# datafusion-contrib/orc-rust

Measured on AMD Instinct MI355X. Metric: decoded GB/s + Mrows/s into Arrow, TPC-H lineitem stripe, higher is better.
Workload: dtype int64/i128/u8

## Files before the change

include/orcgpu.h:

```cpp
#ifndef ORCGPU_H
#define ORCGPU_H

#include <stddef.h>
#include <stdint.h>

#ifdef __cplusplus
extern "C" {
#endif

enum {
  ORCGPU_OK = 0,
  ORCGPU_IO_ERROR = 1,
  ORCGPU_OUT_OF_SPEC = 2,
  ORCGPU_VARINT_TOO_LARGE = 3,
  ORCGPU_DECODE_TIMESTAMP = 4,
  ORCGPU_OFFSET_OVERFLOW = 5,
  ORCGPU_MISMATCHED_SCHEMA = 6,
  ORCGPU_UNSUPPORTED = 7,
  ORCGPU_ARROW = 8,
  ORCGPU_BUILD_DECODER = 9,
  ORCGPU_UNEXPECTED = 10,
  ORCGPU_HIP_ERROR = 100,
  ORCGPU_INVALID_ARGUMENT = 101,
  ORCGPU_END_OF_FILE = 110
// ... 231 lines not shown
int orcgpu_reader_set_device_output(orcgpu_reader* r, int on);
int orcgpu_reader_next_batch_device(orcgpu_reader* r, struct ArrowDeviceArray* out_array, struct ArrowSchema* out_schema);
int orcgpu_reader_d2h_bytes(const orcgpu_reader* r, uint64_t* bytes);
uint64_t orcgpu_result_buffer_bytes(const orcgpu_result* r);
int orcgpu_reader_reads_ahead(orcgpu_reader* r);
int orcgpu_device_array_wait(const struct ArrowDeviceArray* array, void* hip_stream);
int orcgpu_device_array_dlpack(const struct ArrowDeviceArray* array, uint32_t column, int buffer, void** out_managed_tensor);
int orcgpu_unpack_bits(orcgpu_ctx* ctx, const void* d_bits, uint64_t n, uint8_t* d_bytes, void* hip_stream);

#define ORCGPU_ENC_ON_DEVICE 1u
int orcgpu_encode_rle2(orcgpu_ctx* ctx, const void* values, uint64_t n, int int_bytes, int is_signed, uint32_t flags, uint8_t* out, uint64_t out_cap,
                       uint64_t* out_len);
int orcgpu_encode_rle2_i64(orcgpu_ctx* ctx, const int64_t* values, uint64_t n, int is_signed, uint8_t* out, uint64_t out_cap, uint64_t* out_len);
int orcgpu_encode_byte_rle(orcgpu_ctx* ctx, const void* values, uint64_t n, uint32_t flags, uint8_t* out, uint64_t out_cap, uint64_t* out_len);
int orcgpu_encode_boolean(orcgpu_ctx* ctx, const void* bits, uint64_t n_bits, uint32_t flags, uint8_t* out, uint64_t out_cap, uint64_t* out_len);

typedef struct orcgpu_enc_column {
  int32_t arrow_type;
  uint32_t flags;
  uint64_t n_rows;
  const uint8_t* validity;
  const void* values;
  const void* offsets;
} orcgpu_enc_column;
typedef struct orcgpu_enc_stream {
  int32_t kind;
  uint32_t pad;
  const uint8_t* data;
  uint64_t len;
} orcgpu_enc_stream;
int orcgpu_encode_column(orcgpu_ctx* ctx, const orcgpu_enc_column* col, orcgpu_enc_stream streams[3], uint32_t* n_streams);
int orcgpu_encode_fetch(orcgpu_ctx* ctx, const orcgpu_enc_stream* stream, uint8_t* out);

typedef struct orcgpu_writer orcgpu_writer;
typedef struct orcgpu_writer_opts {
  uint32_t batch_size;
  uint32_t pad;
  uint64_t stripe_byte_size;
} orcgpu_writer_opts;
typedef struct orcgpu_writer_counts {
  uint64_t stripes, rows;
  uint64_t bytes;
  uint64_t round_trips;
  uint64_t stripe_round_trips;
  uint64_t nested_slices;
  uint64_t nested_gathers;
} orcgpu_writer_counts;
int orcgpu_writer_open_file(orcgpu_ctx* ctx, const char* path, const struct ArrowSchema* schema, const orcgpu_writer_opts* opts, orcgpu_writer** out);
int orcgpu_writer_open_bytes(orcgpu_ctx* ctx, const struct ArrowSchema* schema, const orcgpu_writer_opts* opts, orcgpu_writer** out);
int orcgpu_writer_write(orcgpu_writer* w, const struct ArrowSchema* schema, const struct ArrowArray* batch, uint32_t flags);
int orcgpu_writer_flush_stripe(orcgpu_writer* w);
int orcgpu_writer_close(orcgpu_writer* w);
int orcgpu_writer_take_bytes(orcgpu_writer* w, uint8_t* out, uint64_t cap, uint64_t* len);
int orcgpu_writer_stats(const orcgpu_writer* w, orcgpu_writer_counts* out);
uint64_t orcgpu_writer_stripe_rows(const orcgpu_writer* w, uint64_t stripe);
void orcgpu_writer_free(orcgpu_writer* w);

int orcgpu_writer_set_compression(orcgpu_writer* w, int kind, uint64_t block_size);
int orcgpu_compress_stream(orcgpu_ctx* ctx, int kind, uint64_t block_size, const void* in, uint64_t n, uint32_t flags, uint8_t* out, uint64_t out_cap,
                           uint64_t* out_len);

int orcgpu_writer_set_row_index(orcgpu_writer* w, uint64_t stride);

int orcgpu_writer_set_dictionary(orcgpu_writer* w, double key_size_threshold);
int orcgpu_writer_dictionary_counts(const orcgpu_writer* w, uint64_t* dictionary, uint64_t* direct);

int orcgpu_writer_set_bloom_filter(orcgpu_writer* w, const char* const* columns, uint32_t n_columns, double fpp);

int orcgpu_last_timing(const orcgpu_ctx* ctx, float* total_ms, float* expand_ms, uint32_t* expand_launches);
#define ORCGPU_N_PHASES 7
int orcgpu_last_phase_ms(const orcgpu_ctx* ctx, float* ms, uint32_t n);

typedef struct orcgpu_lane_stats {
  uint32_t lane, n_lanes;
  uint64_t stream_bytes, arrow_bytes;
  float start_ms, total_ms;
  float phase_ms[ORCGPU_N_PHASES];
  float seq_kernel_ms, exec_kernel_ms;
  float walk_short_kernel_ms, dict_emit_kernel_ms;
  float literals_kernel_ms;
} orcgpu_lane_stats;
int orcgpu_last_lane_stats(const orcgpu_ctx* ctx, uint32_t lane, orcgpu_lane_stats* out);

#ifdef __cplusplus
}
#endif
#endif
```

orc_rust_amd/capi.py:

```python
import ctypes as C
import os

import numpy as np

from . import build as _build

OK = 0
ERR_NAMES = {
    0: "Ok", 1: "IoError", 2: "OutOfSpec", 3: "VarintTooLarge", 4: "DecodeTimestamp", 5: "OffsetOverflow", 6: "MismatchedSchema",
    7: "UnsupportedTypeVariant", 8: "Arrow", 9: "BuildDecoder", 10: "Unexpected", 100: "HipError", 101: "InvalidArgument",
}
COMP = {"none": 0, "zlib": 1, "snappy": 2, "lzo": 3, "lz4": 4, "zstd": 5}
EXPORTS = [
    "orcgpu_open", "orcgpu_close", "orcgpu_last_error", "orcgpu_version", "orcgpu_abi_version", "orcgpu_stage_stripe", "orcgpu_staged_free",
    "orcgpu_staged_bytes", "orcgpu_decode_staged", "orcgpu_stripe_decode", "orcgpu_result_free", "orcgpu_result_status",
    "orcgpu_result_rows", "orcgpu_result_batches", "orcgpu_result_arrow_bytes", "orcgpu_result_batch_view",
    "orcgpu_result_copy_batch", "orcgpu_result_fetch", "orcgpu_result_fetch_async", "orcgpu_result_select", "orcgpu_selection_batches", "orcgpu_timezone_offsets", "orcgpu_result_export_batch", "orcgpu_last_timing", "orcgpu_last_phase_ms", "orcgpu_last_lane_stats", "orcgpu_encode_rle2_i64", "orcgpu_encode_rle2", "orcgpu_encode_byte_rle", "orcgpu_encode_boolean", "orcgpu_encode_column", "orcgpu_encode_fetch",
    "orcgpu_reader_open_file", "orcgpu_reader_open_bytes", "orcgpu_reader_close", "orcgpu_reader_set_batch_size",
    "orcgpu_reader_set_projection", "orcgpu_reader_set_projection_roots", "orcgpu_reader_set_schema", "orcgpu_reader_set_byte_range", "orcgpu_reader_set_shard", "orcgpu_shard_columns", "orcgpu_reader_column_weight", "orcgpu_reader_set_timestamp_precision", "orcgpu_reader_set_row_selection", "orcgpu_reader_set_prefetch",
    "orcgpu_reader_set_row_group_pruning", "orcgpu_reader_row_groups", "orcgpu_index_entry", "orcgpu_reader_set_predicate",
    "orcgpu_predicate_row_groups",
    "orcgpu_result_filter", "orcgpu_reader_set_row_filter", "orcgpu_reader_filter_rows",
    "orcgpu_reader_total_rows", "orcgpu_reader_stripe_count", "orcgpu_reader_column_count", "orcgpu_reader_column_name",
    "orcgpu_reader_next_batch",
    "orcgpu_result_export_batch_device", "orcgpu_reader_set_device_output", "orcgpu_reader_next_batch_device", "orcgpu_reader_d2h_bytes",
    "orcgpu_device_array_wait", "orcgpu_device_array_dlpack", "orcgpu_unpack_bits", "orcgpu_result_buffer_bytes", "orcgpu_reader_reads_ahead",
    "orcgpu_writer_open_file", "orcgpu_writer_open_bytes", "orcgpu_writer_write", "orcgpu_writer_flush_stripe", "orcgpu_writer_close",
    "orcgpu_writer_take_bytes", "orcgpu_writer_stats", "orcgpu_writer_stripe_rows", "orcgpu_writer_free",
    "orcgpu_writer_set_compression", "orcgpu_compress_stream", "orcgpu_writer_set_row_index",
    "orcgpu_writer_set_dictionary", "orcgpu_writer_dictionary_counts",
    "orcgpu_writer_set_bloom_filter",
]


class OrcGpuError(RuntimeError):
    def __init__(self, code, msg=""):
        super().__init__("%s (%d): %s" % (ERR_NAMES.get(code, "?"), code, msg))
        self.code = code


class StreamEntry(C.Structure):
    _fields_ = [("chunk_offset", C.c_uint64), ("skip_bytes", C.c_uint32), ("skip_values", C.c_uint32), ("skip_bits", C.c_uint32)]


class Stream(C.Structure):
    _fields_ = [("column_id", C.c_uint32), ("kind", C.c_int32), ("ptr", C.c_void_p), ("len", C.c_uint64),
                ("skip_bytes", C.c_uint32), ("skip_values", C.c_uint32), ("entries", C.c_void_p), ("n_entries", C.c_uint32), ("skip_bits", C.c_uint32)]


class Column(C.Structure):
    _fields_ = [("column_id", C.c_uint32), ("orc_type", C.c_int32), ("encoding", C.c_int32), ("dictionary_size", C.c_uint32),
                ("precision", C.c_uint32), ("scale", C.c_uint32), ("arrow_target", C.c_int32), ("arrow_precision", C.c_uint32),
                ("arrow_scale", C.c_uint32), ("parent", C.c_uint32)]


class StripeDesc(C.Structure):
    _fields_ = [("n_rows", C.c_uint64), ("compression", C.c_int32), ("block_size", C.c_uint64), ("ts_base_seconds", C.c_int64),
                ("batch_size", C.c_uint32), ("n_streams", C.c_uint32), ("streams", C.POINTER(Stream)), ("n_columns", C.c_uint32),
                ("columns", C.POINTER(Column)), ("writer_timezone", C.c_char_p)]


class LaneStats(C.Structure):
    _fields_ = [("lane", C.c_uint32), ("n_lanes", C.c_uint32), ("stream_bytes", C.c_uint64), ("arrow_bytes", C.c_uint64),
                ("start_ms", C.c_float), ("total_ms", C.c_float), ("phase_ms", C.c_float * 7), ("seq_kernel_ms", C.c_float),
                ("exec_kernel_ms", C.c_float), ("walk_short_kernel_ms", C.c_float), ("dict_emit_kernel_ms", C.c_float),
                ("literals_kernel_ms", C.c_float)]


class RowSelector(C.Structure):
    _fields_ = [("row_count", C.c_uint64), ("skip", C.c_int32)]


def selector_array(selectors):
    arr = (RowSelector * max(1, len(selectors)))()
    for i, (n, skip) in enumerate(selectors):
        arr[i].row_count = n
        arr[i].skip = 1 if skip else 0
    return arr


def selection_batches(selectors, stripe_rows, batch_size=8192):
    L = load()
    cap = len(selectors) + stripe_rows // max(1, batch_size) + 8
    starts, lens = (C.c_uint64 * cap)(), (C.c_uint32 * cap)()
    rest = (RowSelector * (len(selectors) + 2))()
    n_out, n_rest = C.c_uint32(), C.c_uint32()
    rc = L.orcgpu_selection_batches(selector_array(selectors), len(selectors), stripe_rows, batch_size, starts, lens, cap, C.byref(n_out), rest,
                                    len(selectors) + 2, C.byref(n_rest))
    assert rc == 0 and n_out.value <= cap
    return [(starts[i], lens[i]) for i in range(n_out.value)], [(rest[i].row_count, bool(rest[i].skip)) for i in range(n_rest.value)]


def timezone_offsets(name, instants):
    L = load()
    a = np.ascontiguousarray(instants, dtype=np.int64)
    out = np.zeros(len(a), dtype=np.int32)
    epoch = C.c_int64()
    rc = L.orcgpu_timezone_offsets(name.encode(), a.ctypes.data_as(C.c_void_p), len(a), out.ctypes.data_as(C.c_void_p), C.byref(epoch))
    if rc:
        raise OrcGpuError(rc, "time zone %r" % name)
# ... 19 lines not shown


ENC_ON_DEVICE = 1
ARROW = {"bool": 10, "int8": 11, "int16": 12, "int32": 13, "int64": 14, "float32": 15, "float64": 16, "utf8": 17, "binary": 18,
         "large_utf8": 25, "large_binary": 26}


class BatchView(C.Structure):
    _fields_ = [("length", C.c_uint64), ("null_count", C.c_uint64), ("validity", C.c_void_p), ("values", C.c_void_p),
                ("values_bytes", C.c_uint64), ("offsets", C.c_void_p)]


_lib = None
ABI_VERSION = 4


def lib_path():
    return _build.SO


def load():
    global _lib
    if _lib is not None:
        return _lib
    so = os.environ.get("ORCGPU_LIB") or _build.build()
    os.environ.setdefault("GPU_MAX_HW_QUEUES", "8")
    if "TZDIR" not in os.environ and not os.path.isdir("/usr/share/zoneinfo"):
        try:
            import tzdata
            os.environ["TZDIR"] = os.path.join(os.path.dirname(tzdata.__file__), "zoneinfo")
        except ImportError:
            pass
    L = C.CDLL(so)
    L.orcgpu_open.restype = C.c_void_p
    L.orcgpu_open.argtypes = [C.c_int, C.c_void_p]
    L.orcgpu_close.argtypes = [C.c_void_p]
    L.orcgpu_last_error.restype = C.c_char_p
    L.orcgpu_last_error.argtypes = [C.c_void_p]
    L.orcgpu_version.restype = C.c_char_p
    if L.orcgpu_abi_version() != ABI_VERSION:
        raise RuntimeError("liborcgpu.so speaks ABI %d, this binding %d (include/orcgpu.h: ORCGPU_ABI_VERSION)" % (L.orcgpu_abi_version(), ABI_VERSION))
    L.orcgpu_stage_stripe.argtypes = [C.c_void_p, C.POINTER(StripeDesc), C.POINTER(C.c_void_p)]
    L.orcgpu_staged_free.argtypes = [C.c_void_p]
    L.orcgpu_staged_bytes.restype = C.c_uint64
    L.orcgpu_staged_bytes.argtypes = [C.c_void_p]
    L.orcgpu_decode_staged.argtypes = [C.c_void_p, C.POINTER(C.c_void_p), C.c_uint32, C.POINTER(C.c_void_p)]
    L.orcgpu_stripe_decode.argtypes = [C.c_void_p, C.POINTER(StripeDesc), C.POINTER(C.c_void_p)]
    L.orcgpu_result_free.argtypes = [C.c_void_p]
    L.orcgpu_result_status.argtypes = [C.c_void_p, C.POINTER(C.c_uint32), C.POINTER(C.c_uint32)]
    L.orcgpu_result_rows.restype = C.c_uint64
    L.orcgpu_result_rows.argtypes = [C.c_void_p]
    L.orcgpu_result_batches.restype = C.c_uint32
    L.orcgpu_result_batches.argtypes = [C.c_void_p]
    L.orcgpu_result_arrow_bytes.restype = C.c_uint64
    L.orcgpu_result_arrow_bytes.argtypes = [C.c_void_p]
    L.orcgpu_result_batch_view.argtypes = [C.c_void_p, C.c_uint32, C.c_uint32, C.POINTER(BatchView)]
    L.orcgpu_result_copy_batch.argtypes = [C.c_void_p, C.c_void_p, C.c_uint32, C.c_uint32, C.c_void_p, C.c_void_p, C.c_void_p]
    L.orcgpu_result_fetch.argtypes = [C.c_void_p, C.c_void_p]
    L.orcgpu_result_fetch_async.argtypes = [C.c_void_p, C.c_void_p]
    L.orcgpu_reader_set_prefetch.argtypes = [C.c_void_p, C.c_uint32]
    L.orcgpu_reader_set_shard.argtypes = [C.c_void_p, C.c_uint32, C.c_uint32, C.c_int]
    L.orcgpu_shard_columns.argtypes = [C.POINTER(C.c_double), C.c_uint32, C.c_uint32, C.POINTER(C.c_uint32)]
    L.orcgpu_reader_column_weight.argtypes = [C.c_void_p, C.c_uint32]
    L.orcgpu_reader_column_weight.restype = C.c_double
    from .predicate import ColumnIndex, PredicateNode
    L.orcgpu_reader_set_predicate.argtypes = [C.c_void_p, C.POINTER(PredicateNode), C.c_uint32]
    L.orcgpu_predicate_row_groups.argtypes = [C.POINTER(PredicateNode), C.c_uint32, C.POINTER(ColumnIndex), C.c_uint32, C.c_uint64, C.c_uint64,
                                              C.c_void_p, C.POINTER(C.c_uint32)]
    L.orcgpu_result_filter.argtypes = [C.c_void_p, C.c_void_p, C.POINTER(PredicateNode), C.c_uint32, C.POINTER(C.c_char_p), C.c_uint32,
                                       C.POINTER(C.c_uint64)]
    L.orcgpu_reader_set_row_filter.argtypes = [C.c_void_p, C.POINTER(PredicateNode), C.c_uint32]
    L.orcgpu_reader_filter_rows.argtypes = [C.c_void_p, C.POINTER(C.c_uint64), C.POINTER(C.c_uint64)]
    L.orcgpu_reader_set_row_group_pruning.argtypes = [C.c_void_p, C.c_int]
    L.orcgpu_reader_row_groups.argtypes = [C.c_void_p, C.POINTER(C.c_uint64), C.POINTER(C.c_uint64)]
    L.orcgpu_index_entry.argtypes = [C.POINTER(Column), C.c_int, C.c_int, C.POINTER(C.c_uint64), C.c_uint32, C.c_int32, C.POINTER(StreamEntry)]
    L.orcgpu_result_select.argtypes = [C.c_void_p, C.c_void_p, C.POINTER(RowSelector), C.c_uint32]
    L.orcgpu_selection_batches.argtypes = [C.POINTER(RowSelector), C.c_uint32, C.c_uint64, C.c_uint32, C.POINTER(C.c_uint64), C.POINTER(C.c_uint32),
                                           C.c_uint32, C.POINTER(C.c_uint32), C.POINTER(RowSelector), C.c_uint32, C.POINTER(C.c_uint32)]
    L.orcgpu_reader_set_row_selection.argtypes = [C.c_void_p, C.POINTER(RowSelector), C.c_uint32]
    L.orcgpu_result_export_batch.argtypes = [C.c_void_p, C.c_void_p, C.c_uint32, C.c_void_p, C.c_void_p]
    L.orcgpu_last_timing.argtypes = [C.c_void_p, C.POINTER(C.c_float), C.POINTER(C.c_float), C.POINTER(C.c_uint32)]
    L.orcgpu_last_phase_ms.argtypes = [C.c_void_p, C.POINTER(C.c_float), C.c_uint32]
    L.orcgpu_last_lane_stats.argtypes = [C.c_void_p, C.c_uint32, C.POINTER(LaneStats)]
    L.orcgpu_encode_rle2_i64.argtypes = [C.c_void_p, C.c_void_p, C.c_uint64, C.c_int, C.c_void_p, C.c_uint64, C.POINTER(C.c_uint64)]
    L.orcgpu_encode_rle2.argtypes = [C.c_void_p, C.c_void_p, C.c_uint64, C.c_int, C.c_int, C.c_uint32, C.c_void_p, C.c_uint64, C.POINTER(C.c_uint64)]
    L.orcgpu_encode_byte_rle.argtypes = [C.c_void_p, C.c_void_p, C.c_uint64, C.c_uint32, C.c_void_p, C.c_uint64, C.POINTER(C.c_uint64)]
    L.orcgpu_encode_boolean.argtypes = [C.c_void_p, C.c_void_p, C.c_uint64, C.c_uint32, C.c_void_p, C.c_uint64, C.POINTER(C.c_uint64)]
    L.orcgpu_encode_column.argtypes = [C.c_void_p, C.POINTER(EncColumn), C.POINTER(EncStream), C.POINTER(C.c_uint32)]
    L.orcgpu_encode_fetch.argtypes = [C.c_void_p, C.POINTER(EncStream), C.c_void_p]
    L.orcgpu_reader_open_file.argtypes = [C.c_void_p, C.c_char_p, C.POINTER(C.c_void_p)]
    L.orcgpu_reader_open_bytes.argtypes = [C.c_void_p, C.c_char_p, C.c_uint64, C.POINTER(C.c_void_p)]
    L.orcgpu_reader_close.argtypes = [C.c_void_p]
    L.orcgpu_reader_set_batch_size.argtypes = [C.c_void_p, C.c_uint32]
    L.orcgpu_reader_set_projection.argtypes = [C.c_void_p, C.POINTER(C.c_char_p), C.c_uint32]
    L.orcgpu_reader_set_projection_roots.argtypes = [C.c_void_p, C.POINTER(C.c_uint32), C.c_uint32]
    L.orcgpu_reader_set_schema.argtypes = [C.c_void_p, C.c_void_p]
    L.orcgpu_reader_set_byte_range.argtypes = [C.c_void_p, C.c_uint64, C.c_uint64]
    L.orcgpu_reader_set_timestamp_precision.argtypes = [C.c_void_p, C.c_int]
    L.orcgpu_reader_total_rows.restype = C.c_uint64
    L.orcgpu_reader_total_rows.argtypes = [C.c_void_p]
    L.orcgpu_reader_stripe_count.restype = C.c_uint32
    L.orcgpu_reader_stripe_count.argtypes = [C.c_void_p]
    L.orcgpu_reader_column_count.restype = C.c_uint32
    L.orcgpu_reader_column_count.argtypes = [C.c_void_p]
    L.orcgpu_reader_column_name.restype = C.c_char_p
    L.orcgpu_reader_column_name.argtypes = [C.c_void_p, C.c_uint32]
    L.orcgpu_reader_next_batch.argtypes = [C.c_void_p, C.c_void_p, C.c_void_p]
    L.orcgpu_result_export_batch_device.argtypes = [C.c_void_p, C.c_void_p, C.c_uint32, C.c_void_p, C.c_void_p]
    L.orcgpu_reader_set_device_output.argtypes = [C.c_void_p, C.c_int]
    L.orcgpu_reader_next_batch_device.argtypes = [C.c_void_p, C.c_void_p, C.c_void_p]
    L.orcgpu_reader_d2h_bytes.argtypes = [C.c_void_p, C.POINTER(C.c_uint64)]
    L.orcgpu_device_array_wait.argtypes = [C.c_void_p, C.c_void_p]
    L.orcgpu_device_array_dlpack.argtypes = [C.c_void_p, C.c_uint32, C.c_int, C.POINTER(C.c_void_p)]
    L.orcgpu_unpack_bits.argtypes = [C.c_void_p, C.c_void_p, C.c_uint64, C.c_void_p, C.c_void_p]
    L.orcgpu_result_buffer_bytes.restype = C.c_uint64
    L.orcgpu_result_buffer_bytes.argtypes = [C.c_void_p]
    L.orcgpu_reader_reads_ahead.argtypes = [C.c_void_p]
    L.orcgpu_writer_open_file.argtypes = [C.c_void_p, C.c_char_p, C.c_void_p, C.POINTER(WriterOpts), C.POINTER(C.c_void_p)]
    L.orcgpu_writer_open_bytes.argtypes = [C.c_void_p, C.c_void_p, C.POINTER(WriterOpts), C.POINTER(C.c_void_p)]
    L.orcgpu_writer_write.argtypes = [C.c_void_p, C.c_void_p, C.c_void_p, C.c_uint32]
    L.orcgpu_writer_flush_stripe.argtypes = [C.c_void_p]
    L.orcgpu_writer_close.argtypes = [C.c_void_p]
    L.orcgpu_writer_take_bytes.argtypes = [C.c_void_p, C.c_void_p, C.c_uint64, C.POINTER(C.c_uint64)]
    L.orcgpu_writer_stats.argtypes = [C.c_void_p, C.POINTER(WriterCounts)]
    L.orcgpu_writer_stripe_rows.restype = C.c_uint64
    L.orcgpu_writer_stripe_rows.argtypes = [C.c_void_p, C.c_uint64]
    L.orcgpu_writer_free.argtypes = [C.c_void_p]
    L.orcgpu_writer_set_compression.argtypes = [C.c_void_p, C.c_int, C.c_uint64]
    L.orcgpu_writer_set_row_index.argtypes = [C.c_void_p, C.c_uint64]
    L.orcgpu_writer_set_dictionary.argtypes = [C.c_void_p, C.c_double]
    L.orcgpu_writer_dictionary_counts.argtypes = [C.c_void_p, C.POINTER(C.c_uint64), C.POINTER(C.c_uint64)]
    L.orcgpu_writer_set_bloom_filter.argtypes = [C.c_void_p, C.POINTER(C.c_char_p), C.c_uint32, C.c_double]
    L.orcgpu_compress_stream.argtypes = [C.c_void_p, C.c_int, C.c_uint64, C.c_void_p, C.c_uint64, C.c_uint32, C.c_void_p, C.c_uint64,
                                         C.POINTER(C.c_uint64)]
    _lib = L
    return L


class Context:

    def __init__(self, device=0):
        self.L = load()
        self.device = device
        self.h = self.L.orcgpu_open(device, None)
        if not self.h:
            raise OrcGpuError(100, "orcgpu_open(%d) failed: no usable HIP device (this library has no CPU path)" % device)

    def close(self):
        if self.h:
            self.L.orcgpu_close(self.h)
            self.h = None

    def __del__(self):
        try:
            self.close()
        except Exception:
            pass

    def error(self):
        return self.L.orcgpu_last_error(self.h).decode("utf-8", "replace")

    def _check(self, rc):
        if rc:
            raise OrcGpuError(rc, self.error())

    def stage(self, n_rows, streams, columns, compression="none", block_size=262144, batch_size=8192, ts_base=0, writer_timezone=None):
# ... 67 lines not shown
        n = len(data)
        bound = C.c_uint64(0)
        self._check(self.L.orcgpu_compress_stream(self.h, kind, block_size, v.ctypes.data, n, 0, None, 0, C.byref(bound)))
        out = np.zeros(max(1, bound.value), dtype=np.uint8)
        m = C.c_uint64(0)
        self._check(self.L.orcgpu_compress_stream(self.h, kind, block_size, v.ctypes.data, n, 0, out.ctypes.data, out.size, C.byref(m)))
        return out[:m.value].tobytes()

    def compress_stream_device(self, d_in, n, codec, d_out, out_cap, block_size=262144):
        kind = COMP[codec] if isinstance(codec, str) else codec
        m = C.c_uint64(0)
        self._check(self.L.orcgpu_compress_stream(self.h, kind, block_size, d_in, n, ENC_ON_DEVICE, d_out, out_cap, C.byref(m)))
        return m.value

    def encode_column(self, arrow_type, n_rows, values, validity=None, offsets=None):
        keep = [np.ascontiguousarray(values)]
        col = EncColumn(ARROW[arrow_type], 0, n_rows, None, keep[0].ctypes.data if keep[0].size else None, None)
        if keep[0].size == 0:
            keep.append(np.zeros(1, dtype=np.uint8))
            col.values = keep[-1].ctypes.data
        if validity is not None:
            keep.append(np.ascontiguousarray(validity, dtype=np.uint8))
            if keep[-1].size == 0:
                keep[-1] = np.zeros(1, dtype=np.uint8)
            col.validity = keep[-1].ctypes.data
        if offsets is not None:
            keep.append(np.ascontiguousarray(offsets))
            col.offsets = keep[-1].ctypes.data
        streams = (EncStream * 3)()
        n = C.c_uint32(0)
        self._check(self.L.orcgpu_encode_column(self.h, C.byref(col), streams, C.byref(n)))
        out = []
        for i in range(n.value):
            buf = np.zeros(max(1, streams[i].len), dtype=np.uint8)
            self._check(self.L.orcgpu_encode_fetch(self.h, C.byref(streams[i]), buf.ctypes.data))
            out.append((streams[i].kind, buf[:streams[i].len].tobytes()))
        return out

    def decode(self, staged_list, results=None):
        n = len(staged_list)
        sarr = (C.c_void_p * n)(*[s.h for s in staged_list])
        rarr = (C.c_void_p * n)(*[(r.h if r is not None else None) for r in (results or [None] * n)])
        self._check(self.L.orcgpu_decode_staged(self.h, sarr, n, rarr))
        return [results[i] if results and results[i] is not None else Result(self, rarr[i]) for i in range(n)]

    def result_filter(self, result, predicate, column_names):
        nodes, keep = predicate.flatten()
        names = (C.c_char_p * max(1, len(column_names)))(*[n.encode() for n in column_names])
        kept = C.c_uint64(0)
        self._check(self.L.orcgpu_result_filter(self.h, result.h, nodes, len(nodes), names, len(column_names), C.byref(kept)))
        return kept.value

    def timing(self):
        a, b, c = C.c_float(), C.c_float(), C.c_uint32()
        self.L.orcgpu_last_timing(self.h, C.byref(a), C.byref(b), C.byref(c))
        return a.value, b.value, c.value


    PHASES = ("decompress", "walk", "present", "expand", "finish")

    def phase_ms(self):
        a = (C.c_float * 7)()
        self.L.orcgpu_last_phase_ms(self.h, a, 7)
        return dict(zip(self.PHASES + ("decompress_stage1", "decompress_tables"), [float(x) for x in a]))

    def lane_stats(self):
        out = []
        k = 0
        while True:
            st = LaneStats()
            if self.L.orcgpu_last_lane_stats(self.h, k, C.byref(st)) != OK:
                break
            out.append({"lane": st.lane, "n_lanes": st.n_lanes, "stream_bytes": int(st.stream_bytes), "arrow_bytes": int(st.arrow_bytes),
                        "start_ms": float(st.start_ms), "total_ms": float(st.total_ms),
                        "phase_ms": dict(zip(self.PHASES + ("decompress_stage1", "decompress_tables"), [float(x) for x in st.phase_ms])),
                        "seq_kernel_ms": float(st.seq_kernel_ms), "exec_kernel_ms": float(st.exec_kernel_ms),
                        "walk_short_kernel_ms": float(st.walk_short_kernel_ms), "dict_emit_kernel_ms": float(st.dict_emit_kernel_ms),
                        "literals_kernel_ms": float(st.literals_kernel_ms)})
            k += 1
            if k >= st.n_lanes:
                break
        return out


class Staged:
    def __init__(self, ctx, h):
        self.ctx, self.h = ctx, h

    def nbytes(self):
        return self.ctx.L.orcgpu_staged_bytes(self.h)

    def free(self):
        if self.h:
            self.ctx.L.orcgpu_staged_free(self.h)
            self.h = None

    def __del__(self):
        try:
            self.free()
        except Exception:
            pass


class Result:
    def __init__(self, ctx, h):
        self.ctx, self.h = ctx, h

    def free(self):
        if self.h:
            self.ctx.L.orcgpu_result_free(self.h)
            self.h = None

    def __del__(self):
        try:
            self.free()
        except Exception:
            pass

    def status(self):
        b, c = C.c_uint32(), C.c_uint32()
        st = self.ctx.L.orcgpu_result_status(self.h, C.byref(b), C.byref(c))
        return st, b.value, c.value

    @property
    def rows(self):
        return self.ctx.L.orcgpu_result_rows(self.h)

    @property
    def n_batches(self):
        return self.ctx.L.orcgpu_result_batches(self.h)

    @property
    def arrow_bytes(self):
        return self.ctx.L.orcgpu_result_arrow_bytes(self.h)

    @property
    def buffer_bytes(self):
        return self.ctx.L.orcgpu_result_buffer_bytes(self.h)

    def view(self, batch, column):
        v = BatchView()
        self.ctx._check(self.ctx.L.orcgpu_result_batch_view(self.h, batch, column, C.byref(v)))
        return v

    def batch(self, batch, column):
        v = self.view(batch, column)
        n = v.length
        values = np.zeros(max(1, v.values_bytes), dtype=np.uint8)
        offsets = np.zeros(n + 1, dtype=np.int32) if v.offsets else None
        validity = np.zeros((n + 7) // 8, dtype=np.uint8) if v.validity else None
        self.ctx._check(self.ctx.L.orcgpu_result_copy_batch(
            self.ctx.h, self.h, batch, column, values.ctypes.data, offsets.ctypes.data if offsets is not None else None,
            validity.ctypes.data if validity is not None else None))
        return {"status": 0, "length": n, "null_count": v.null_count, "validity": validity.tobytes() if validity is not None else None,
                "values": values[:v.values_bytes].tobytes(), "offsets": offsets}

    def select(self, selectors):
        self.ctx._check(self.ctx.L.orcgpu_result_select(self.ctx.h, self.h, selector_array(selectors), len(selectors)))

    def fetch(self):
        self.ctx._check(self.ctx.L.orcgpu_result_fetch(self.ctx.h, self.h))

    def fetch_async(self):
        self.ctx._check(self.ctx.L.orcgpu_result_fetch_async(self.ctx.h, self.h))

    def export_batch_device(self, batch):
# ... 15 lines not shown
```

orc_rust_amd/csrc/device/decompress_kernels.hip:

```cpp
#pragma once
#include "rle_parse.h"

struct ChunkDesc {
  const uint8_t* src;
  uint8_t* dst;
  uint8_t* scratch;
  uint32_t src_len;
  uint32_t dst_cap;
  uint32_t kind;
  uint32_t stream;
  uint32_t out_len;
  uint32_t status;
  uint32_t first_item, n_items;
  uint32_t diag;
  uint32_t pad;
};

struct StreamDesc {
  uint32_t first_chunk, n_chunks;
  uint32_t len_idx;
  uint32_t err_idx;
  uint8_t* base;
  uint32_t framing_error;
  uint32_t skip;
};

__device__ __forceinline__ void wave_fence() { __builtin_amdgcn_fence(__ATOMIC_SEQ_CST, "workgroup"); }
__device__ __forceinline__ void lds_order() {
  __builtin_amdgcn_fence(__ATOMIC_ACQ_REL, "wavefront");
  __builtin_amdgcn_wave_barrier();
}

__device__ __forceinline__ void st_u64(uint8_t* p, uint64_t v) { __builtin_memcpy(p, &v, 8); }

__device__ __forceinline__ void wave_copy(uint8_t* dst, const uint8_t* src, uint32_t n, uint32_t lane) {
  uint32_t k = lane * 8;
  for (; k + 8 <= n; k += 512) st_u64(dst + k, ld_u64(src + k));
  uint32_t done = n & ~7u;
  for (uint32_t t = done + lane; t < n; t += 64) dst[t] = src[t];
}

__device__ __forceinline__ void wave_match(uint8_t* dst, uint64_t out, uint32_t off, uint32_t len, uint32_t lane) {
  const uint8_t* s = dst + out - off;
  uint8_t* d = dst + out;
  if (off >= len) {
    if (off >= 8 && len >= 64) {
      uint32_t k = lane * 8;
      for (; k + 8 <= len; k += 512) st_u64(d + k, ld_u64(s + k));
      for (uint32_t t = (len & ~7u) + lane; t < len; t += 64) d[t] = s[t];
    } else {
      for (uint32_t k = lane; k < len; k += 64) d[k] = s[k];
    }
  } else {
    for (uint32_t k = lane; k < len; k += 64) d[k] = s[k % off];
  }
}

#define LZ_FLUSH 4096u
#define LZ_STAGE 4096u
template <uint32_t RING>
struct LzStore {
  uint8_t ring[RING];
  uint8_t stage[LZ_STAGE + 16];
};
struct LzLds {
  uint8_t* ring;
  uint32_t rsize;
  uint8_t* stage;
};
template <uint32_t RING>
__device__ __forceinline__ LzLds lz_view(LzStore<RING>& s) {
  return LzLds{s.ring, RING, s.stage};
}
struct LzOut {
  uint8_t* ring;
  uint32_t rmask;
  uint8_t* dst;
  uint64_t out;
  uint64_t flushed;
};
__device__ __forceinline__ void lz_flush(LzOut& o, uint32_t lane) {
  lds_order();
  const uint32_t n = (uint32_t)(o.out - o.flushed);
  for (uint32_t k = lane * 8; k < n; k += 512) {
    const uint32_t ri = (uint32_t)(o.flushed + k) & o.rmask;
    if (k + 8 <= n && ri + 8 <= o.rmask + 1) {
      uint64_t v;
      __builtin_memcpy(&v, o.ring + ri, 8);
      st_u64(o.dst + o.flushed + k, v);
    } else {
      for (uint32_t t = k; t < n && t < k + 8; t++) o.dst[o.flushed + t] = o.ring[(uint32_t)(o.flushed + t) & o.rmask];
    }
  }
  o.flushed = o.out;
}
__device__ __forceinline__ void lz_maybe_flush(LzOut& o, uint32_t lane) {
  if (o.out - o.flushed >= LZ_FLUSH) lz_flush(o, lane);
}
__device__ __forceinline__ void lz_byte(LzOut& o, uint32_t b, uint32_t lane) {
  if (lane == 0) o.ring[(uint32_t)o.out & o.rmask] = (uint8_t)b;
  o.out++;
  lz_maybe_flush(o, lane);
}
__device__ __forceinline__ void lz_literal(LzOut& o, const uint8_t* src, uint32_t len, uint32_t lane) {
  for (uint32_t done = 0; done < len;) {
    const uint32_t piece = len - done < LZ_FLUSH ? len - done : LZ_FLUSH;
    for (uint32_t k = lane; k < piece; k += 64) o.ring[(uint32_t)(o.out + k) & o.rmask] = src[done + k];
    o.out += piece;
// ... 195 lines not shown
```

orc_rust_amd/csrc/device/lz_exec.h:

```cpp
#pragma once

#ifndef LZX_STAGE
#define LZX_STAGE 8192u
#endif
#ifndef LZX_STAGE_WAVE
#define LZX_STAGE_WAVE 2048u
#endif
#define LZX_DONE 0xffffu
#define LZX_WATCHDOG 25000u
#define LZX_SEQ_PACKED 0xffffffffu
#define LZX_DEFERRED 0x57a7u

struct ZItem {
  uint32_t kind;
  uint32_t flags;
  uint32_t size;
  uint32_t src_off;
  uint32_t lit_kind;
  uint32_t lit_off, litn, nseq;
  uint32_t zblock;
  uint32_t seq_packed;
  uint64_t fcs;
  uint32_t ck_off;
  uint32_t pad;
};

template <int T>
struct ExecLds {
  static constexpr uint32_t STAGE = T <= 64 ? LZX_STAGE_WAVE : LZX_STAGE;
  __attribute__((aligned(16))) uint8_t stage[STAGE + 64];
  __attribute__((aligned(16))) uint16_t ptr[STAGE + 64];
  uint64_t wsum[T / 64];
  uint32_t wred[T / 64];
  uint32_t wrep[T / 64][6];
  uint32_t ilit[T > 64 ? T : 1];
  uint32_t sdst[T > 64 ? T : 1];
  uint32_t lsrc[T > 64 ? T : 1];
  uint32_t bc[16];
  uint32_t big[8][3];
};

struct RepX {
  uint32_t t0, v0, t1, v1, t2, v2;
};
__device__ __forceinline__ RepX rep_identity() { return RepX{0, 0, 1, 0, 2, 0}; }
__device__ __forceinline__ void rep_pick(const RepX& f, uint32_t tag, uint32_t& t, uint32_t& v) {
  t = tag == 0 ? f.t0 : (tag == 1 ? f.t1 : f.t2);
  v = tag == 0 ? f.v0 : (tag == 1 ? f.v1 : f.v2);
}
__device__ __forceinline__ void rep_expr(const RepX& f, uint32_t gt, uint32_t gv, uint32_t& t, uint32_t& v) {
  if (gt == 3) {
    t = 3;
    v = gv;
  } else {
    uint32_t ft, fv;
    rep_pick(f, gt, ft, fv);
    t = ft;
    v = ft == 3 ? fv - gv : fv + gv;
  }
}
__device__ __forceinline__ RepX rep_compose(const RepX& g, const RepX& f) {
  RepX r;
  rep_expr(f, g.t0, g.v0, r.t0, r.v0);
  rep_expr(f, g.t1, g.v1, r.t1, r.v1);
  rep_expr(f, g.t2, g.v2, r.t2, r.v2);
  return r;
}
__device__ __forceinline__ RepX rep_of_sequence(uint32_t ofv, uint32_t ll) {
  if (ofv > 3) return RepX{3, ofv - 3, 0, 0, 1, 0};
  const uint32_t idx = ofv - 1 + (ll == 0 ? 1u : 0u);
  if (idx == 0) return rep_identity();
  if (idx == 1) return RepX{1, 0, 0, 0, 2, 0};
  if (idx == 2) return RepX{2, 0, 0, 0, 1, 0};
  return RepX{0, 1, 0, 0, 1, 0};
}
template <int CTRL, int ROWS>
__device__ __forceinline__ RepX rep_dpp(const RepX& x) {
  RepX r;
  r.t0 = (uint32_t)__builtin_amdgcn_update_dpp(0, (int)x.t0, CTRL, ROWS, 0xf, false);
  r.v0 = (uint32_t)__builtin_amdgcn_update_dpp(0, (int)x.v0, CTRL, ROWS, 0xf, false);
  r.t1 = (uint32_t)__builtin_amdgcn_update_dpp(1, (int)x.t1, CTRL, ROWS, 0xf, false);
  r.v1 = (uint32_t)__builtin_amdgcn_update_dpp(0, (int)x.v1, CTRL, ROWS, 0xf, false);
  r.t2 = (uint32_t)__builtin_amdgcn_update_dpp(2, (int)x.t2, CTRL, ROWS, 0xf, false);
  r.v2 = (uint32_t)__builtin_amdgcn_update_dpp(0, (int)x.v2, CTRL, ROWS, 0xf, false);
  return r;
}
__device__ __forceinline__ RepX rep_wave_scan(RepX x) {
  x = rep_compose(x, rep_dpp<0x111, 0xf>(x));
  x = rep_compose(x, rep_dpp<0x112, 0xf>(x));
  x = rep_compose(x, rep_dpp<0x114, 0xf>(x));
  x = rep_compose(x, rep_dpp<0x118, 0xf>(x));
  x = rep_compose(x, rep_dpp<0x142, 0xa>(x));
  x = rep_compose(x, rep_dpp<0x143, 0xc>(x));
  return x;
}

__device__ __forceinline__ void lds_iota16(uint16_t* p, uint32_t v0, uint32_t n) {
  uint64_t pat = (uint64_t)v0 * 0x0001000100010001ull + 0x0003000200010000ull;
  uint32_t k = 0;
  for (; k + 4 <= n; k += 4, pat += 0x0004000400040004ull) __builtin_memcpy(p + k, &pat, 8);
  if (n & 2u) {
    const uint32_t x = (uint32_t)pat;
    __builtin_memcpy(p + k, &x, 4);
    k += 2;
    pat >>= 32;
  }
  if (n & 1u) p[k] = (uint16_t)pat;
}
// ... 704 lines not shown
```

orc_rust_amd/csrc/device/zstd_entropy.h:

```cpp
#pragma once

struct ZBlock {
  const uint8_t* src;
  uint8_t* lit_out;
  uint32_t* seq_out;
  uint32_t chunk;
  uint32_t content_off, content_end;
  uint32_t lit_type, lit_streams, lit_hdr, lit_regen, lit_comp;
  uint32_t nseq, seq_off;
  uint32_t huf_off, huf_end;
  uint32_t tab_off[3];
  uint32_t tab_end[3];
  uint32_t pad[2];
};

struct ZSeqHdr {
  uint32_t bit_off;
  uint32_t logs;
  uint32_t status;
  uint32_t pad;
};
__device__ __forceinline__ uint2 zseq_pack(uint32_t ofv, uint32_t ml, uint32_t ll) {
  const uint32_t o = ofv < 0x1fffffffu ? ofv : 0x1fffffffu;
  return make_uint2(o | ml << 29, ml >> 3 | ll << 15);
}
__device__ __forceinline__ void zseq_unpack(uint2 p, uint32_t& ofv, uint32_t& ml, uint32_t& ll) {
  ofv = p.x & 0x1fffffffu;
  ml = p.x >> 29 | (p.y & 0x7fffu) << 3;
  ll = p.y >> 15;
}
#define ZL_CELLS 1280u
#define ZL_LL 0u
#define ZL_ML 512u
#define ZL_OF 1024u

struct ZFse {
  uint16_t next;
  uint8_t nb;
  uint8_t add;
  uint32_t base;
};

struct ZEntLds {
  union {
    struct {
      uint16_t huf[2048];
      uint8_t weights[256];
      FseEnt wt[64];
    } h;
    struct {
      __attribute__((aligned(16))) uint8_t lit_pad[4096 + 256 + 64 * 8];
      __attribute__((aligned(16))) uint8_t chunk[64 * ZL_CHUNK];
    };
    struct {
      ZFse ll[512], ml[512], of[256];
      ZFse zero;
      union {
        struct {
          uint32_t seqbuf[64 * 3 + 64];
          __attribute__((aligned(8))) uint8_t bits[2048 + 16];
        };
        __attribute__((aligned(16))) uint16_t ctab[1280];
      };
    } s;
  };
  int16_t norm[256];
  uint16_t next[256];
  uint8_t sym[512];
  __attribute__((aligned(4))) uint8_t stage[208];
};

__device__ __forceinline__ int zfse_build(ZFse* t, uint8_t* symtab, const int16_t* norm, int nsym, int log, uint16_t* next, int which, uint32_t lane,
                                          uint16_t* ct = nullptr) {
  const uint32_t size = 1u << log;
  const uint32_t step = (size >> 1) + (size >> 3) + 3, mask = size - 1;
  const int cnt = (int)lane < nsym ? (int)norm[lane] : 0;
  const bool low = cnt == -1;
  const unsigned long long lowm = __ballot(low);
  const unsigned long long below = (1ull << lane) - 1;
  const uint32_t nlow = (uint32_t)__popcll(lowm);
  const uint32_t c = cnt > 0 ? (uint32_t)cnt : 0u;
  const uint32_t incl = wave_incl_scan_u32(c, lane);
  if ((uint32_t)__builtin_amdgcn_readlane((int)incl, 63) + nlow != size) return 1;
  const uint32_t high = size - 1 - nlow;
  uint8_t* expand = reinterpret_cast<uint8_t*>(next);
  if (low) symtab[size - 1 - (uint32_t)__popcll(lowm & below)] = (uint8_t)lane;
  for (uint32_t k = incl - c; k < incl; k++) expand[k] = (uint8_t)lane;
  wave_sync();
  uint32_t placed = 0;
  for (uint32_t t0 = 0; t0 < size; t0 += 64) {
    const uint32_t tt = t0 + lane;
    const uint32_t u = (tt * step) & mask;
    const bool f = tt < size && u <= high;
    const unsigned long long m = __ballot(f);
    if (f) symtab[u] = expand[placed + (uint32_t)__popcll(m & below)];
    placed += (uint32_t)__popcll(m);
  }
  wave_sync();
  const uint32_t my_add = which == 0 ? (lane < 36 ? Z_LL_BITS[lane] : 0u) : (which == 1 ? lane : (lane < 53 ? Z_ML_BITS[lane] : 0u));
  const uint32_t my_base = which == 0 ? (lane < 36 ? Z_LL_BASE[lane] : 0u) : (which == 1 ? 1u << (lane & 31u) : (lane < 53 ? Z_ML_BASE[lane] : 0u));
  uint32_t nxt = low ? 1u : c;
  for (uint32_t i0 = 0; i0 < size; i0 += 64) {
    const uint32_t i = i0 + lane;
    const bool valid = i < size;
// ... 549 lines not shown
```

orc_rust_amd/csrc/orcgpu.hip:

```cpp
#include <hip/hip_runtime.h>

#include <algorithm>
#include <chrono>
#include <atomic>
#include <condition_variable>
#include <deque>
#include <functional>
#include <map>
#include <memory>
#include <mutex>
#include <thread>
#include <sys/mman.h>
#include <cmath>
#include <cstdarg>
#include <cstdio>
#include <cstring>
#include <string>
#include <vector>

#include "../../include/orcgpu.h"
#include "device/rle_kernels.h"
#include "device/rle_parse.h"
#include "device/rle_scan.hip"
#include "device/rle_expand.hip"
#include "device/multi_job.h"
#include "device/column_kernels.hip"
#include "device/string_kernels.hip"
#include "device/decompress_kernels.hip"
#include "device/select_kernels.hip"
#include "device/filter_kernels.hip"
#include "device/rle_encode.hip"
#include "device/lz_compress.hip"
#include "device/writer_types.hip"
#include "device/writer_dict.hip"
#include "device/writer_nested.hip"
#include "device/col_stats.hip"
#include "device/bloom_build.hip"
#include "device/export_kernels.hip"

#include "arrow_c_data.h"
#include "../../include/orcgpu_dlpack.h"
#include "device_hold.h"

namespace {

constexpr uint64_t kAlign = 256;
constexpr int kWalkRounds = 4;
inline uint64_t align_up(uint64_t v, uint64_t a = kAlign) { return (v + a - 1) / a * a; }

struct DevBuf {
  uint8_t* p = nullptr;
  size_t cap = 0;
  bool ensure(size_t n) {
    if (n <= cap) return true;
    if (p) (void)hipFree(p);
    p = nullptr;
    cap = 0;
    size_t want = n + n / 8 + (1u << 20);
    if (hipMalloc((void**)&p, want) != hipSuccess) {
      if (hipMalloc((void**)&p, n) != hipSuccess) return false;
      want = n;
    }
    cap = want;
    return true;
  }
  void release() {
    if (p) (void)hipFree(p);
    p = nullptr;
    cap = 0;
  }
};

struct Bump {
  uint64_t off = 0;
  uint64_t take(uint64_t n, uint64_t a = kAlign) {
    off = align_up(off, a);
    uint64_t r = off;
    off += n;
    return r;
  }
};

struct ChunkInfo {
  uint64_t src_off;
  uint32_t len;
  uint32_t original;
  uint32_t plain_cap;
  int32_t zparse = -1;
};


}

#include "orcgpu_zstd_host.inc"
#include "orcgpu_tz.inc"

namespace {
struct StagedStream {
  uint32_t column_id;
  int32_t kind;
  uint64_t off;
  uint64_t len;
  std::vector<ChunkInfo> chunks;
  std::vector<ZChunkParse> zchunks;
  uint32_t skip_bytes = 0, skip_values = 0, skip_bits = 0;
  std::vector<std::pair<uint32_t, uint32_t>> hints;
  bool framing_error = false;
  uint64_t framed_len = 0;
};
}

constexpr int kMaxLanes = 4;
constexpr uint64_t kZstdLanesMinSequences = 40000000ull;
constexpr size_t kStagePiece = 16u << 20;
constexpr int kCopyThreads = 6;

struct CopyPool {
  struct Task {
    uint8_t* dst;
    const uint8_t* src;
    size_t n;
  };
  std::vector<std::thread> threads;
  std::mutex m;
  std::condition_variable cv, done;
  std::vector<Task> tasks;
  size_t next = 0, pending = 0;
  bool stop = false;
  CopyPool() {
    int n = kCopyThreads;
    if (const char* e = getenv("ORCGPU_STAGE_THREADS")) n = std::max(0, std::min(64, atoi(e)));
    for (int i = 0; i < n; i++) threads.emplace_back([this] { run(); });
  }
  ~CopyPool() {
    {
      std::lock_guard<std::mutex> g(m);
      stop = true;
    }
    cv.notify_all();
    for (auto& t : threads) t.join();
  }
  void run() {
    for (;;) {
      Task t;
      {
        std::unique_lock<std::mutex> g(m);
        cv.wait(g, [this] { return stop || next < tasks.size(); });
        if (stop) return;
        t = tasks[next++];
      }
      if (t.src) memcpy(t.dst, t.src, t.n);
      else memset(t.dst, 0, t.n);
      {
        std::lock_guard<std::mutex> g(m);
        if (--pending == 0) done.notify_all();
      }
    }
  }
  void copy_all(std::vector<Task>& ts) {
    size_t total = 0;
    for (auto& t : ts) total += t.n;
    if (total < (1u << 20)) {
      for (auto& t : ts) {
        if (t.src) memcpy(t.dst, t.src, t.n);
        else memset(t.dst, 0, t.n);
      }
      return;
    }
    std::vector<Task> sl;
    for (auto& t : ts)
      for (size_t o = 0; o < t.n; o += 1u << 20) sl.push_back(Task{t.dst + o, t.src ? t.src + o : nullptr, std::min<size_t>(1u << 20, t.n - o)});
    {
      std::lock_guard<std::mutex> g(m);
      tasks.swap(sl);
      next = 0;
      pending = tasks.size();
    }
    cv.notify_all();
    for (;;) {
      Task t;
      {
        std::lock_guard<std::mutex> g(m);
        if (next >= tasks.size()) break;
        t = tasks[next++];
      }
      if (t.src) memcpy(t.dst, t.src, t.n);
      else memset(t.dst, 0, t.n);
      std::lock_guard<std::mutex> g(m);
      if (--pending == 0) done.notify_all();
    }
    std::unique_lock<std::mutex> g(m);
    done.wait(g, [this] { return pending == 0; });
    tasks.clear();
    next = 0;
  }
};

struct orcgpu_ctx {
  int device = 0;
  int lane_id = 0;
  orcgpu_ctx* lanes[kMaxLanes] = {nullptr, nullptr, nullptr, nullptr};
  hipStream_t stream = nullptr;
  std::string err;
  DevBuf scratch;
  DevBuf enc_a, enc_b, enc_in, enc_tmp, enc_out[3];
  DevBuf lzc_tab, lzc_stage, lzc_io;
  uint8_t* pinned = nullptr;
  size_t pinned_cap = 0;
  uint8_t* fin_pinned = nullptr;
  size_t fin_pinned_cap = 0;
  hipEvent_t ev[10] = {nullptr, nullptr, nullptr, nullptr, nullptr, nullptr, nullptr, nullptr, nullptr, nullptr};
  uint32_t n_cus = 0;
  uint32_t dbg_inflate_threads = 0, dbg_exec_threads = 0;
  hipEvent_t kev[2][2] = {{nullptr, nullptr}, {nullptr, nullptr}};
  bool kev_used[2] = {false, false};
  hipStream_t aux_stream = nullptr;
  hipEvent_t aux_ev[2] = {nullptr, nullptr};
  bool exact_on = false;
  hipEvent_t lit_ev[2] = {nullptr, nullptr};
  bool lit_ev_used = false;
  float last_total_ms = 0, last_expand_ms = 0;
  float last_phase_ms[ORCGPU_N_PHASES] = {0, 0, 0, 0, 0, 0, 0};
  orcgpu_lane_stats last_stats{};
  uint32_t last_n_lanes = 1;
  double call_t0 = 0;
  orcgpu_ctx* gate_peers[kMaxLanes] = {nullptr, nullptr, nullptr, nullptr};
  int n_gate_peers = 0;
int call_z_lanes = -1;
    std::atomic<int> tables_gate{0};
  uint32_t last_expand_launches = 0;
  hipStream_t copy_stream = nullptr;
  hipStream_t d2h_stream = nullptr;
  hipEvent_t d2h_gate = nullptr;
  uint8_t* piece[2] = {nullptr, nullptr};
  hipEvent_t piece_ev[2] = {nullptr, nullptr};
  bool piece_used[2] = {false, false};
  int piece_next = 0;
  std::vector<std::pair<uint8_t*, size_t>> arena_pool;
  std::mutex pool_m;
  std::mutex err_m;
  struct CopyPool* copiers = nullptr;
  struct Zone {
    TzTable table;
    uint8_t* dev = nullptr;
    int64_t epoch = 1420070400;
  };
  std::map<std::string, std::shared_ptr<Zone>> zones;
  std::vector<std::pair<uint8_t*, size_t>> up_blocks;
  size_t up_block = 0, up_off = 0;
  void upload_reset() { up_block = up_off = 0; }
  hipError_t upload(void* dst, const void* src, size_t n, hipStream_t st) {
    if (!n) return hipSuccess;
    const size_t need = (n + 63) & ~(size_t)63;
    while (up_block < up_blocks.size() && up_off + need > up_blocks[up_block].second) up_block++, up_off = 0;
    if (up_block == up_blocks.size()) {
      uint8_t* b = nullptr;
      const size_t cap = std::max<size_t>(2 * need, 1u << 20);
      hipError_t e = hipHostMalloc((void**)&b, cap, hipHostMallocDefault);
      if (e != hipSuccess) return e;
      up_blocks.push_back({b, cap});
      up_off = 0;
    }
    uint8_t* h = up_blocks[up_block].first + up_off;
    up_off += need;
    memcpy(h, src, n);
    return hipMemcpyAsync(dst, h, n, hipMemcpyHostToDevice, st);
  }
  bool ensure_pinned(size_t n) {
    if (n <= pinned_cap) return true;
    if (pinned) (void)hipHostFree(pinned);
    pinned = nullptr;
    pinned_cap = 0;
    size_t want = n + n / 4 + (1u << 16);
    if (hipHostMalloc((void**)&pinned, want, hipHostMallocDefault) != hipSuccess) return false;
    pinned_cap = want;
    return true;
  }
};

struct orcgpu_staged {
  orcgpu_ctx* ctx = nullptr;
  orcgpu_stripe_desc desc{};
  std::vector<orcgpu_column> cols;
  std::vector<StagedStream> streams;
  uint8_t* dev = nullptr;
  size_t dev_bytes = 0;
  size_t dev_cap = 0;
  hipEvent_t ready = nullptr;
  std::shared_ptr<orcgpu_ctx::Zone> zone;
  uint64_t stream_bytes = 0;
  bool has_sel = false;
  std::vector<SelBatch> sel;
  bool piece = false;
  const StagedStream* find(uint32_t col, int kind) const {
    for (auto& s : streams)
      if (s.column_id == col && s.kind == kind) return &s;
    return nullptr;
  }
};

namespace {

struct ColumnOut {
  int32_t orc_type = 0;
  uint32_t column_id = 0;
  uint32_t width = 0;
  bool is_string = false, is_bool = false;
  bool is_struct = false;
// ... 132 lines not shown
  std::vector<std::string> field_names;
  std::vector<orcgpu_result*> subs;
  std::vector<uint32_t> src_col;
  int status = 0;
  uint32_t err_batch = 0, err_col = 0;
  uint64_t arrow_bytes = 0;
};

namespace {

void set_err(orcgpu_ctx* c, const char* fmt, ...) {
  char buf[512];
  va_list ap;
  va_start(ap, fmt);
  vsnprintf(buf, sizeof(buf), fmt, ap);
  va_end(ap);
  if (c) {
    std::lock_guard<std::mutex> g(c->err_m);
    c->err = buf;
  }
}

#define HIP_TRY(ctx, expr)                                                              \
  do {                                                                                  \
    hipError_t e_ = (expr);                                                             \
    if (e_ != hipSuccess) {                                                             \
      set_err(ctx, "%s failed: %s (%s:%d)", #expr, hipGetErrorString(e_), __FILE__, __LINE__); \
      return ORCGPU_HIP_ERROR;                                                          \
    }                                                                                   \
  } while (0)

void scan_chunks(const uint8_t* ptr, uint64_t len_total, int compression, uint64_t block_size, StagedStream& st) {
  uint64_t p = 0;
  while (p < len_total) {
    if (p + 3 > len_total) {
      st.framing_error = true;
      break;
    }
    uint32_t h = (uint32_t)ptr[p] | ((uint32_t)ptr[p + 1] << 8) | ((uint32_t)ptr[p + 2] << 16);
    uint32_t len = h >> 1;
    if (p + 3 + len > len_total) {
      st.framing_error = true;
      break;
    }
    uint32_t cap = (uint32_t)block_size;
    if (h & 1) {
      cap = len;
    } else if (compression == ORCGPU_COMP_SNAPPY) {
      uint64_t u = 0;
      int shift = 0;
      for (uint32_t k = 0; k < len && k < 5; k++) {
        uint8_t c = ptr[p + 3 + k];
        u |= (uint64_t)(c & 0x7f) << shift;
        shift += 7;
        if (!(c & 0x80)) break;
      }
      cap = (uint32_t)std::min<uint64_t>(u, std::max<uint64_t>(block_size, 1u << 22));
    }
    ChunkInfo ci{p + 3, len, h & 1, cap, -1};
    if (!(h & 1) && compression == ORCGPU_COMP_ZSTD) {
      ZChunkParse zp;
      zstd_parse_chunk(ptr + p + 3, len, zp);
      const uint64_t limit = std::max<uint64_t>(block_size, 1u << 22);
      const uint64_t bound = zp.size_known ? zp.plain_size : limit;
      uint64_t need_seq = 0, need_lit = 0;
      for (auto& it : zp.items) {
        need_seq += it.kind == 2 ? 3ull * it.nseq : 0;
        need_lit += it.kind == 2 ? it.lit_regen : 0;
      }
      if (!zp.bad && (bound > limit || need_seq > bound || need_lit > bound)) zp.bad = true;
      if (zp.bad) {
        zp.items.clear();
        ci.plain_cap = 0;
      } else if (zp.size_known) {
        ci.plain_cap = (uint32_t)zp.plain_size;
      }
      ci.zparse = (int32_t)st.zchunks.size();
      st.zchunks.push_back(std::move(zp));
    }
    st.chunks.push_back(ci);
    p += 3 + (uint64_t)len;
  }
  st.framed_len = p;
}

uint32_t type_width(int t) {
  switch (t) {
    case ORCGPU_T_BYTE: return 1;
    case ORCGPU_T_SHORT: return 2;
    case ORCGPU_T_INT:
    case ORCGPU_T_DATE:
    case ORCGPU_T_FLOAT: return 4;
    case ORCGPU_T_LONG:
    case ORCGPU_T_DOUBLE:
    case ORCGPU_T_TIMESTAMP:
    case ORCGPU_T_TIMESTAMP_INSTANT: return 8;
    case ORCGPU_T_DECIMAL: return 16;
    default: return 0;
  }
}
bool is_string_type(int t) { return t == ORCGPU_T_STRING || t == ORCGPU_T_VARCHAR || t == ORCGPU_T_CHAR || t == ORCGPU_T_BINARY; }

constexpr int kMaxStructDepth = 256;
constexpr int kMaxTypeDepth = 256;
enum JobClass { JC_PRESENT = 0, JC_RLE2 = 1, JC_RLE1 = 2, JC_BYTE = 3, JC_PRESENT1 = 4, JC_COUNT = JC_PRESENT1 + kMaxStructDepth };

struct JobPlan {
  int cls;
  uint8_t codec, is_signed, nbits, out_bytes;
  const uint8_t* data;
  uint64_t data_scratch_off = ~0ull;
  uint64_t len_upper;
  uint32_t len_idx, needed_idx, total_idx;
  uint64_t out_scratch_off = ~0ull;
  uint64_t out_result_off = ~0ull;
  int result_index = 0;
  uint64_t expect_values;
  uint32_t block0 = 0, nblocks = 0, group0 = 0, ngroups = 0, group_size = 64;
  uint32_t skip_values = 0;
  const StagedStream* hint_src = nullptr;
  uint32_t chunk0 = 0;
  uint32_t uniform_idx = 0, uniform_value = 0;
  int stripe = 0, col = 0, role = 0;
  int final_index = -1;
};

struct PlainStream {
  const uint8_t* dev = nullptr;
  uint64_t scratch_off = ~0ull;
  uint64_t len_upper = 0;
  uint32_t len_idx = 0;
  uint32_t err_idx = 0;
  uint32_t skip_values = 0;
  uint32_t skip_bits = 0;
  const StagedStream* src = nullptr;
  uint32_t chunk0 = 0;
  bool exists = false;
  bool in_result = false;
};

constexpr int ORCGPU_RETRY_LARGER_SLOTS = 1000;

struct DecompStream {
  const orcgpu_staged* stripe;
  const StagedStream* st;
  uint64_t scratch_off;
  uint32_t len_idx, err_idx;
  int result_index = -1;
  uint64_t result_off = 0;
};

struct ColPlan {
  int stripe, col;
  orcgpu_column c;
  uint64_t n_rows;
  bool has_present = false;
  bool own_present = false;
  int parent_plan = -1;
  int depth = 0;
  uint32_t ceil8_idx = 0;
  uint32_t nonascii_idx = 0;
  uint32_t uniform_idx = 0;
  uint32_t child_bits = 0;
  bool child_bits_set = false;
  int arm0 = -1, n_arms = 0;
  int arm_of = -1, arm_tag = 0;
// ... 520 lines not shown
```

orc_rust_amd/csrc/orcgpu_decode.inc:

```

namespace {

int ts_unit_of(const orcgpu_column& c) {
  switch (c.arrow_target) {
    case ORCGPU_ARROW_TIMESTAMP_S: case ORCGPU_ARROW_TIMESTAMP_S_UTC: case ORCGPU_ARROW_TIMESTAMP_S_NOTZ: return 0;
    case ORCGPU_ARROW_TIMESTAMP_MS: case ORCGPU_ARROW_TIMESTAMP_MS_UTC: case ORCGPU_ARROW_TIMESTAMP_MS_NOTZ: return 1;
    case ORCGPU_ARROW_TIMESTAMP_US: case ORCGPU_ARROW_TIMESTAMP_US_UTC: case ORCGPU_ARROW_TIMESTAMP_US_NOTZ: return 2;
    case ORCGPU_ARROW_DECIMAL128: return 4;
    default: return 3;
  }
}

int schema_pair_status(const orcgpu_column& c) {
  const int a = c.arrow_target;
  if (a == ORCGPU_ARROW_DEFAULT) return 0;
  const bool unit_default = a >= ORCGPU_ARROW_TIMESTAMP_S && a <= ORCGPU_ARROW_TIMESTAMP_NS;
  switch (c.orc_type) {
    case ORCGPU_T_BOOLEAN: return a == ORCGPU_ARROW_BOOLEAN ? 0 : ORCGPU_MISMATCHED_SCHEMA;
    case ORCGPU_T_BYTE: return a == ORCGPU_ARROW_INT8 ? 0 : ORCGPU_MISMATCHED_SCHEMA;
    case ORCGPU_T_SHORT: return a == ORCGPU_ARROW_INT16 ? 0 : ORCGPU_MISMATCHED_SCHEMA;
    case ORCGPU_T_INT: return a == ORCGPU_ARROW_INT32 ? 0 : ORCGPU_MISMATCHED_SCHEMA;
    case ORCGPU_T_LONG: return a == ORCGPU_ARROW_INT64 ? 0 : ORCGPU_MISMATCHED_SCHEMA;
    case ORCGPU_T_FLOAT: return a == ORCGPU_ARROW_FLOAT32 ? 0 : ORCGPU_MISMATCHED_SCHEMA;
    case ORCGPU_T_DOUBLE: return a == ORCGPU_ARROW_FLOAT64 ? 0 : ORCGPU_MISMATCHED_SCHEMA;
// ... 402 lines not shown
    if (!P.results[si]->arena[ctx->lane_id].ensure(P.result_bump[si].off + kAlign)) {
      set_err(ctx, "hipMalloc(%llu) for the result buffers failed", (unsigned long long)P.result_bump[si].off);
      return ORCGPU_HIP_ERROR;
    }
  }
  if (!ctx->ensure_pinned(SL.bytes + DP.table_bytes + 64)) {
    set_err(ctx, "hipHostMalloc for the summary failed");
    return ORCGPU_HIP_ERROR;
  }
  uint8_t* S = ctx->scratch.p;
  {
    static const char* poison = getenv("ORCGPU_POISON");
    if (poison && *poison) {
      const int v = (int)strtol(poison, nullptr, 0) & 0xFF;
      (void)hipMemsetAsync(S, v, P.scratch.off, st);
      for (uint32_t si = 0; si < n; si++) (void)hipMemsetAsync(P.results[si]->arena[ctx->lane_id].p, v, P.result_bump[si].off, st);
    }
  }
  uint8_t* hs = ctx->pinned;
  memset(hs, 0, SL.bytes);
  memcpy(hs + SL.scalars_off, P.scalars.data(), P.scalars.size() * 8);
  RleJob* hjobs = reinterpret_cast<RleJob*>(hs + SL.jobs_off);
  for (size_t k = 0; k < order.size(); k++) {
    const JobPlan& j = P.jobs[order[k]];
    RleJob& d = hjobs[k];
    d.data = j.data_scratch_off != ~0ull ? S + j.data_scratch_off : j.data;
    d.out = j.out_result_off != ~0ull ? (void*)(P.results[j.result_index]->arena[ctx->lane_id].p + j.out_result_off) : (void*)(S + j.out_scratch_off);
    d.len_idx = j.len_idx;
    d.needed_idx = j.needed_idx;
    d.total_idx = j.total_idx;
    d.block0 = j.block0;
    d.nblocks = j.nblocks;
    d.group0 = j.group0;
    d.ngroups = j.ngroups;
    d.group_size = j.group_size;
    d.group_tab0 = cls_tab0[j.cls] + j.group0;
    d.class_index = (uint32_t)j.final_index - cls_first[j.cls];
    d.codec = j.codec;
    d.is_signed = j.is_signed;
    d.nbits = j.nbits;
    d.out_bytes = j.out_bytes;
    d.first_bad = 0xffffffffu;
    d.stat_bad = 0;
    d.stat_repaired = 0;
    d.skip = j.skip_values;
    d.bad_left = 0;
    d.hint0 = d.n_hints = d.hint_bad = 0;
    d.hint_skip = j.hint_src ? j.hint_src->skip_bytes : 0;
    d.uniform_idx = j.uniform_idx;
    d.uniform_value = j.uniform_value;
    d.err = RLE_NO_ERR;
    d.err_pos = RLE_NO_ERR;
  }
  for (size_t h = 0; h < hints.size(); h++) {
    RleJob& d = hjobs[hints[h].job];
    if (!d.n_hints) d.hint0 = (uint32_t)h;
    d.n_hints++;
  }
  uint8_t* dsum = S + summary_off;
  uint64_t* d_scalars = reinterpret_cast<uint64_t*>(dsum + SL.scalars_off);
  RleJob* d_jobs = reinterpret_cast<RleJob*>(dsum + SL.jobs_off);
  unsigned long long* d_nullc = reinterpret_cast<unsigned long long*>(dsum + SL.nullc_off);
  unsigned long long* d_chartot = reinterpret_cast<unsigned long long*>(dsum + SL.chartot_off);
  RleBlocks blk;
  blk.entry = reinterpret_cast<uint32_t*>(S + blk_entry);
  blk.exit_ = reinterpret_cast<uint32_t*>(S + blk_exit);
  blk.nvals = reinterpret_cast<uint32_t*>(S + blk_nvals);
  blk.voff = reinterpret_cast<uint32_t*>(S + blk_voff);
  blk.tile_base = reinterpret_cast<uint32_t*>(S + blk_tbase);
  blk.flags = S + blk_flags;
  blk.badmap = reinterpret_cast<uint32_t*>(S + blk_badmap);
  blk.group_job = reinterpret_cast<uint32_t*>(S + blk_gjob);
  blk.hint = hints.empty() ? nullptr : reinterpret_cast<uint32_t*>(S + blk_hint);
  uint32_t* d_tsum = reinterpret_cast<uint32_t*>(S + blk_tsum);
  const int njobs = (int)order.size();

  ht_plan = hclock();
  for (uint32_t si = 0; si < n; si++)
    if (stripes[si]->ready) HIP_TRY(ctx, hipStreamWaitEvent(st, stripes[si]->ready, 0));
  HIP_TRY(ctx, hipEventRecord(ctx->ev[0], st));
  ctx->kev_used[0] = ctx->kev_used[1] = false;
  ctx->lit_ev_used = false;
  HIP_TRY(ctx, hipMemcpyAsync(dsum, hs, SL.bytes, hipMemcpyHostToDevice, st));
  rc = launch_decompress(ctx, P, DP, S, d_scalars, hs + SL.bytes, ctx->ev[6], ctx->ev[7], ctx->ev[4], ctx->ev[8]);
  const double ht_first = hclock();
  if (rc) return rc;
  if (njobs && !hints.empty()) {
    HIP_TRY(ctx, hipMemsetAsync(blk.hint, 0xff, total_blocks * 4, st));
    HIP_TRY(ctx, ctx->upload(S + hints_off, hints.data(), hints.size() * sizeof(RleHint), st));
    HIP_TRY(ctx, launch(rle_hint_kernel, (uint64_t)hints.size(), false, 64, st, d_jobs, (const RleHint*)(S + hints_off), (uint32_t)hints.size(), blk,
                        (const uint64_t*)d_scalars, (const uint32_t*)(DP.n_chunks ? S + DP.chunk_start_off : S)));
  }
  if (njobs) {
    static const int kModes[] = {0, 3, -1, 1, 1, 2};
    for (int mode : kModes) {
      if (mode < 0)
      {
        uint32_t spw = 1;
        while (spw < 8 && total_blocks / (64ull * spw * 2) >= 2048) spw *= 2;
        if (!ctx->kev_used[0]) HIP_TRY(ctx, hipEventRecord(ctx->kev[0][0], st));
        HIP_TRY(ctx, launch(rle_walk_short_kernel, (total_blocks + 64ull * spw - 1) / (64ull * spw), true, 64 * RLE_SHORT_WAVES, st, d_jobs, njobs, blk,
                            (const uint64_t*)d_scalars, (uint32_t)total_blocks, spw));
        HIP_TRY(ctx, hipEventRecord(ctx->kev[0][1], st));
        ctx->kev_used[0] = true;
      }
      else
        HIP_TRY(ctx, launch(rle_walk_kernel, total_blocks, false, 64, st, d_jobs, njobs, blk, (const uint64_t*)d_scalars, (uint32_t)total_blocks, mode));
    }
    constexpr int mend_passes = 2;
    for (int pass = 0; pass < mend_passes; pass++) {
      HIP_TRY(ctx, launch(rle_mend_kernel, total_blocks, false, 256, st, d_jobs, njobs, blk, (const uint64_t*)d_scalars, (uint32_t)total_blocks));
      HIP_TRY(ctx, launch(rle_walk_kernel, total_blocks, false, 64, st, d_jobs, njobs, blk, (const uint64_t*)d_scalars, (uint32_t)total_blocks, 5));
    }
    if (use_exact && mend_passes > 0) {
      uint16_t* fmap = reinterpret_cast<uint16_t*>(S + x_fmap);
      uint16_t* gmap = reinterpret_cast<uint16_t*>(S + x_gmap);
      uint32_t* tile_e = reinterpret_cast<uint32_t*>(S + x_tile);
      uint32_t* span_e = reinterpret_cast<uint32_t*>(S + x_span);
      const uint64_t cus = ctx->n_cus ? ctx->n_cus : 256;
      HIP_TRY(ctx, launch(rle_exact_map_kernel, std::min<uint64_t>(n_xspans, 2 * cus), true, RLE_EXACT_WG, st, d_jobs, njobs, (const uint64_t*)d_scalars, (uint32_t)total_blocks, fmap));
      HIP_TRY(ctx, launch(rle_exact_tile_kernel, std::min<uint64_t>(n_tiles, 4 * cus), true, RLE_EXACT_WG, st, d_jobs, njobs, (const uint64_t*)d_scalars, (uint32_t)total_blocks,
                          (const uint16_t*)fmap, gmap));
      HIP_TRY(ctx, launch(rle_exact_chain_kernel, (uint64_t)njobs, true, 64, st, d_jobs, njobs, (const uint64_t*)d_scalars, (const uint16_t*)fmap, (const uint16_t*)gmap, tile_e, span_e));
      HIP_TRY(ctx, launch(rle_exact_fill_kernel, std::min<uint64_t>(n_xspans, 2 * cus), true, RLE_EXACT_WG, st, d_jobs, njobs, blk, (const uint64_t*)d_scalars, (uint32_t)total_blocks,
                          (const uint32_t*)span_e));
    }
    HIP_TRY(ctx, launch(rle_repair_kernel, (uint64_t)njobs, true, 64, st, d_jobs, njobs, blk, (const uint64_t*)d_scalars));
    HIP_TRY(ctx, launch(rle_tile_scan_kernel, (uint64_t)n_tiles, true, 256, st, blk, d_tsum));
    HIP_TRY(ctx, launch(rle_job_scan_kernel, (uint64_t)njobs, true, 256, st, (const RleJob*)d_jobs, blk, (const uint32_t*)d_tsum, d_scalars));
  }
  HIP_TRY(ctx, hipEventRecord(ctx->ev[5], st));
  const double ht_walk = hclock();
  {
    size_t pres_at = 0;
    P.presjobs.reserve(P.cols.size());
    PresJob* const dp_all = reinterpret_cast<PresJob*>(S + P.presjobs_off);
    P.presjobs.clear();
    int max_depth = 0;
    for (auto& cp : P.cols) max_depth = std::max(max_depth, cp.depth);
    for (int depth = 0; depth <= max_depth && depth <= kMaxStructDepth; depth++) {
      const int cls = depth == 0 ? JC_PRESENT : JC_PRESENT1 + depth - 1;
      if (cls_groups[cls])
        HIP_TRY(ctx, launch(byte_expand_kernel, (uint64_t)(cls_groups[cls] + 3) / 4, true, 256, st, d_jobs + cls_first[cls],
                            (const uint32_t*)(blk.group_job + cls_tab0[cls]), blk, (const uint64_t*)d_scalars, cls_groups[cls]));
      uint64_t max_words = 0, max_tiles = 0, max_out = 0;
      for (auto& cp : P.cols) {
        if (!cp.has_present || cp.depth != depth || !cp.n_rows) continue;
        orcgpu_result* r = P.results[cp.stripe];
        PresJob j{};
        if (cp.arm_of >= 0) {
          const ColPlan& un = P.cols[cp.arm_of];
          j.tags = reinterpret_cast<const int8_t*>(S + un.dense_off);
          j.tag = cp.arm_tag;
          j.child_bits = cp.child_bits;
          j.vbits = reinterpret_cast<unsigned long long*>(S + cp.vbits_off);
          j.wpop = reinterpret_cast<uint32_t*>(S + cp.wpop_off);
          j.rank = reinterpret_cast<uint32_t*>(S + cp.rank_off);
          j.rtiles = reinterpret_cast<uint32_t*>(S + cp.rank_tiles_off);
          j.validity = reinterpret_cast<unsigned long long*>(S + cp.arm_validity_off);
          j.null_counts = d_nullc + cp.nullcount_off;
          j.nonnull_out = d_scalars + cp.nonnull_idx;
          j.ceil8b_out = d_scalars + cp.ceil8_idx;
          if (un.has_present) {
            j.parent_vbits = reinterpret_cast<const unsigned long long*>(S + un.vbits_off);
            j.parent_rank = reinterpret_cast<const uint32_t*>(S + un.rank_off);
          }
// ... 176 lines not shown
    HIP_TRY(ctx, hipMemcpyAsync(dj, hj, bytes, hipMemcpyHostToDevice, st));
    k = 0;
    for (auto& e : fin.entries) {
      e.launcher(dj + k, (uint32_t)e.jobs.size(), e.max_blocks, st);
      k += e.jobs.size();
    }
    HIP_TRY(ctx, hipGetLastError());
  }
  for (auto& j : tzjobs) HIP_TRY(ctx, launch(tz_shift_kernel, j.n_rows, false, 256, st, j));
  if (!P.spacejobs.empty()) {
    const uint32_t ns = (uint32_t)P.spacejobs.size();
    SpaceJob* ds = reinterpret_cast<SpaceJob*>(S + P.spacejobs_off);
    uint64_t max_rows = 0;
    for (auto& j : P.spacejobs) max_rows = std::max(max_rows, j.n_rows);
    HIP_TRY(ctx, ctx->upload(ds, P.spacejobs.data(), ns * sizeof(SpaceJob), st));
    for (uint32_t o = 0; o < ns; o += 65535u)
      hipLaunchKernelGGL(space_multi_kernel, dim3((uint32_t)((max_rows + 255) / 256), std::min<uint32_t>(65535u, ns - o)), dim3(256), 0, st,
                         (const SpaceJob*)(ds + o));
    HIP_TRY(ctx, hipGetLastError());
  }
  const double ht_fin = hclock();
  rc = launch_dict_rows(ctx, P, S, d_scalars, d_chartot);
  if (rc) return rc;
  const double ht_dict = hclock();
  rc = launch_post_ext(ctx, P, S, dsum, hs, SL, d_chartot);
  if (rc) return rc;
  HIP_TRY(ctx, launch(summary_to_host_kernel, (uint64_t)(SL.bytes / 8), false, 256, st, (const unsigned long long*)dsum, (unsigned long long*)hs,
                      (uint64_t)(SL.bytes / 8)));
  HIP_TRY(ctx, hipEventRecord(ctx->ev[3], st));
  ht_enq = hclock();
  HIP_TRY(ctx, hipStreamSynchronize(st));
  rc = settle_dict_places(ctx, P, S, dsum, hs, SL);
  if (rc) return rc;
  ht_sync = hclock();
  if (host_prof) {
    fprintf(stderr, "[orcgpu] lane %d host us: plan %.1f (columns %.1f, chunk tables %.1f, jobs %.1f)  first launch after %.1f  enqueue %.1f  wait %.1f\n", ctx->lane_id, ht_plan - ht0, ht_cols - ht0, ht_dp - ht_cols, ht_plan - ht_dp, ht_first - ht0, ht_enq - ht_plan, ht_sync - ht_enq);
    fprintf(stderr, "[orcgpu] lane %d enqueue us: decompress %.1f  walk %.1f  present %.1f  expand %.1f  finishers %.1f  dictionary rows %.1f  post %.1f\n", ctx->lane_id,
            ht_first - ht_plan, ht_walk - ht_first, ht_pres - ht_walk, ht_exp - ht_pres, ht_fin - ht_exp, ht_dict - ht_fin, ht_enq - ht_dict);
  }
  (void)hipEventElapsedTime(&ctx->last_total_ms, ctx->ev[0], ctx->ev[3]);
  (void)hipEventElapsedTime(&ctx->last_expand_ms, ctx->ev[1], ctx->ev[2]);
  {
    static const int edge[6] = {0, 4, 5, 1, 2, 3};
    for (int k = 0; k < 5; k++) (void)hipEventElapsedTime(&ctx->last_phase_ms[k], ctx->ev[edge[k]], ctx->ev[edge[k + 1]]);
    (void)hipEventElapsedTime(&ctx->last_phase_ms[5], ctx->ev[0], ctx->ev[6]);
    (void)hipEventElapsedTime(&ctx->last_phase_ms[6], ctx->ev[0], ctx->ev[7]);
    {
      orcgpu_lane_stats& ls = ctx->last_stats;
      ls = orcgpu_lane_stats{};
      ls.lane = (uint32_t)ctx->lane_id;
      ls.n_lanes = 1;
      for (uint32_t si = 0; si < n; si++)
        for (size_t ci = 0; ci < stripes[si]->cols.size(); ci++) {
          if (mask && !(*mask)[si][ci]) continue;
          for (auto& sst : stripes[si]->streams)
            if (sst.column_id == stripes[si]->cols[ci].column_id) ls.stream_bytes += sst.len;
        }
      ls.start_ms = (float)((ht_plan - (ctx->call_t0 > 0 ? ctx->call_t0 : ht0)) * 1e-3);
      ls.total_ms = ctx->last_total_ms;
      for (int k = 0; k < ORCGPU_N_PHASES; k++) ls.phase_ms[k] = ctx->last_phase_ms[k];
      if (DP.z_lanes && DP.n_zchains && DP.n_chunks) (void)hipEventElapsedTime(&ls.seq_kernel_ms, ctx->ev[9], ctx->ev[8]);
      ls.exec_kernel_ms = ctx->last_phase_ms[0] - ctx->last_phase_ms[5];
      if (ctx->lit_ev_used && hipEventSynchronize(ctx->lit_ev[1]) == hipSuccess) (void)hipEventElapsedTime(&ls.literals_kernel_ms, ctx->lit_ev[0], ctx->lit_ev[1]);
      if (ctx->kev_used[0]) (void)hipEventElapsedTime(&ls.walk_short_kernel_ms, ctx->kev[0][0], ctx->kev[0][1]);
      if (ctx->kev_used[1] && hipEventSynchronize(ctx->kev[1][1]) == hipSuccess) (void)hipEventElapsedTime(&ls.dict_emit_kernel_ms, ctx->kev[1][0], ctx->kev[1][1]);
    }
    if (host_prof)
      fprintf(stderr, "[orcgpu] lane %d GPU ms: decompress %.3f  walk %.3f  present %.3f  expand %.3f  finish %.3f  (total %.3f)\n", ctx->lane_id, ctx->last_phase_ms[0],
              ctx->last_phase_ms[1], ctx->last_phase_ms[2], ctx->last_phase_ms[3], ctx->last_phase_ms[4], ctx->last_total_ms);
  }

  {
    bool want = false;
    for (int k = 0; k < njobs && !want; k++) want = hjobs[k].bad_left >= 32u;
    ctx->exact_on = want;
  }
  if (getenv("ORCGPU_DEBUG"))
    for (int k = 0; k < njobs; k++)
      fprintf(stderr, "[orcgpu] job %d (stripe %d col %d role %d block0 %u nbits %d) codec %d blocks %u group %u: bad %u (first %u) repaired %u total %llu\n", k, P.jobs[order[k]].stripe, P.jobs[order[k]].col, P.jobs[order[k]].role, hjobs[k].block0, (int)hjobs[k].nbits, hjobs[k].codec, hjobs[k].nblocks,
              hjobs[k].group_size, hjobs[k].stat_bad, hjobs[k].first_bad, hjobs[k].stat_repaired, (unsigned long long)reinterpret_cast<const uint64_t*>(hs + SL.scalars_off)[hjobs[k].total_idx]);
  if (getenv("ORCGPU_DEBUG") && DP.n_zitems) {
    fprintf(stderr, "[orcgpu] zstd plan: %u blocks, %u with sequences (%llu in all): %s\n", DP.n_zblocks, DP.n_zchains, (unsigned long long)DP.z_total_seq,
            DP.z_lanes ? "one lane per block" : "one wavefront per block");
    std::vector<std::pair<uint64_t, uint32_t>> top;
    for (uint32_t c = 0; c < DP.n_chunks; c++) {
      uint64_t ns = 0;
      const uint32_t f = DP.chunk_first_item[c], e = c + 1 < DP.n_chunks ? DP.chunk_first_item[c + 1] : DP.n_zitems;
      for (uint32_t k = f; k < e; k++) ns += DP.zitems[k].item->nseq;
      top.push_back({ns, c});
    }
    std::sort(top.rbegin(), top.rend());
    {
      size_t h40 = 0, h20 = 0, h10 = 0, h5 = 0;
      for (auto& t : top) h40 += t.first >= 40000, h20 += t.first >= 20000, h10 += t.first >= 10000, h5 += t.first >= 5000;
      fprintf(stderr, "[orcgpu] zstd chunks: %zu; with >= 40k / 20k / 10k / 5k sequences: %zu / %zu / %zu / %zu\n", top.size(), h40, h20, h10, h5);
    }
    for (size_t k = 0; k < top.size() && k < 6; k++) {
      const uint32_t c = top[k].second, f = DP.chunk_first_item[c], e = c + 1 < DP.n_chunks ? DP.chunk_first_item[c + 1] : DP.n_zitems;
      uint32_t mxs = 0, lit = 0;
      for (uint32_t q = f; q < e; q++) mxs = std::max(mxs, DP.zitems[q].item->nseq), lit += DP.zitems[q].item->lit_regen;
      fprintf(stderr, "[orcgpu] zstd chunk %u: %u blocks, %llu sequences (largest block %u), %u literal bytes\n", c, e - f, (unsigned long long)top[k].first, mxs, lit);
    }
  }
  if (getenv("ORCGPU_DEBUG") && DP.n_chunks) {
    std::vector<uint8_t> tb(DP.table_bytes);
    (void)hipMemcpy(tb.data(), S + DP.dev_off, DP.table_bytes, hipMemcpyDeviceToHost);
    const ChunkDesc* cc = reinterpret_cast<const ChunkDesc*>(tb.data() + DP.chunks_off);
    const ZBlock* zz = reinterpret_cast<const ZBlock*>(tb.data() + DP.zblocks_off);
    std::vector<uint32_t> zs(2 * DP.n_zblocks + 1);
    if (DP.n_zblocks) (void)hipMemcpy(zs.data(), S + DP.zstatus_off, 8ull * DP.n_zblocks, hipMemcpyDeviceToHost);
    uint32_t shown = 0;
    {
      uint32_t pend = 0, wd = 0;
      for (uint32_t k = 0; k < 2 * DP.n_zblocks; k++) pend += zs[k] == 0xffffffffu, wd += zs[k] == 0x57a7u;
      if (pend || wd) fprintf(stderr, "[orcgpu] entropy jobs: %u of %u still pending, %u watchdog\n", pend, 2 * DP.n_zblocks, wd);
    }
    {
      uint32_t n_deflate = 0, n_deferred = 0, n_exec_bad = 0;
      for (uint32_t k = 0; k < DP.n_chunks; k++)
        if (cc[k].kind == 1) n_deflate++, n_deferred += cc[k].diag == LZX_DEFERRED, n_exec_bad += cc[k].diag != LZX_DEFERRED && cc[k].diag != 0;
      if (n_deflate)
        fprintf(stderr, "[orcgpu] deflate: %u chunks of %u in the call, token stage %u threads per chunk, execution %u threads per chunk, %u deferred to the serial decoder, %u rejected by the execution kernel\n",
                n_deflate, DP.n_chunks, ctx->dbg_inflate_threads, ctx->dbg_exec_threads, n_deferred, n_exec_bad);
    }
    for (uint32_t k = 0; k < DP.n_chunks && shown < 16; k++)
      if (cc[k].status) fprintf(stderr, "[orcgpu] chunk %u (stream %u, kind %u, %u bytes, cap %u): rejected, diag %u\n", k, cc[k].stream, cc[k].kind, cc[k].src_len, cc[k].dst_cap, cc[k].diag), shown++;
    for (uint32_t k = 0; k < DP.n_zblocks && shown < 32; k++)
      if (zs[k] | zs[DP.n_zblocks + k]) fprintf(stderr, "[orcgpu] zstd block %u (chunk %u, nseq %u, lit type %u regen %u): entropy stage code %u\n", k, zz[k].chunk, zz[k].nseq, zz[k].lit_type, zz[k].lit_regen, zs[k] ? zs[k] : zs[DP.n_zblocks + k]), shown++;
  }
#ifdef ORC_PROF
  if (getenv("ORCGPU_DEBUG")) {
    unsigned long long hp[176];
    hipMemcpyFromSymbol(hp, HIP_SYMBOL(g_prof), sizeof(hp));
    static const struct { int base; const char* who; } sect[] = {{0, "walk"}, {48, "decompress"}, {80, "lz_exec"}, {112, "zstd_entropy"}};
    for (auto& sc : sect)
      for (int k = 0; k < 16; k++)
        if (hp[sc.base + 2 * k]) fprintf(stderr, "[orcgpu] prof %s phase %d: sum %.1f us  max %.2f us\n", sc.who, k, hp[sc.base + 2 * k] * 0.01, hp[sc.base + 2 * k + 1] * 0.01);
    for (int k = 32; k < 48; k++)
      if (hp[k]) fprintf(stderr, "[orcgpu] prof counter %d: %llu\n", k, hp[k]);
    for (int k = 144; k < 176; k++)
      if (hp[k]) fprintf(stderr, "[orcgpu] prof counter %d: %llu\n", k, hp[k]);
    memset(hp, 0, sizeof(hp));
    hipMemcpyToSymbol(HIP_SYMBOL(g_prof), hp, sizeof(hp));
  }
#endif
  {
    bool codec_error = false;
    const uint64_t* hsc = reinterpret_cast<const uint64_t*>(hs + SL.scalars_off);
    for (auto& ds : P.decomp) codec_error = codec_error || hsc[ds.err_idx] != 0;
    if (codec_error && DP.n_chunks) {
      std::vector<ChunkDesc> hc(DP.n_chunks);
      HIP_TRY(ctx, hipMemcpy(hc.data(), S + DP.dev_off + DP.chunks_off, (size_t)DP.n_chunks * sizeof(ChunkDesc), hipMemcpyDeviceToHost));
      bool grown = false;
      uint32_t ci = 0;
      for (auto& ds : P.decomp) {
        const int kind = ds.stripe->desc.compression;
        const uint64_t limit = std::max<uint64_t>(ds.stripe->desc.block_size, 1u << 22);
        for (auto& c : const_cast<StagedStream*>(ds.st)->chunks) {
          const bool grows = kind == ORCGPU_COMP_ZLIB || kind == ORCGPU_COMP_LZO ||
                             (kind == ORCGPU_COMP_ZSTD && c.zparse >= 0 && !ds.st->zchunks[c.zparse].size_known && !ds.st->zchunks[c.zparse].bad);
          if (!c.original && grows && hc[ci].status && c.plain_cap < limit) {
            c.plain_cap = (uint32_t)limit;
            grown = true;
          }
          ci++;
        }
      }
      if (grown) return ORCGPU_RETRY_LARGER_SLOTS;
    }
  }
  const uint64_t* h_scalars = reinterpret_cast<const uint64_t*>(hs + SL.scalars_off);
  const unsigned long long* h_nullc = reinterpret_cast<const unsigned long long*>(hs + SL.nullc_off);
  const unsigned long long* h_chartot = reinterpret_cast<const unsigned long long*>(hs + SL.chartot_off);
  for (auto& cp : P.cols) {
    if (cp.col < 0) continue;
    orcgpu_result* r = P.results[cp.stripe];
    ColumnOut& co = r->cols[cp.col];
    for (uint32_t b = 0; b < r->n_batches; b++) co.null_counts[b] = cp.has_present || cp.tz ? h_nullc[cp.nullcount_off + b] : 0;
    auto batch_of_dense = [&](uint64_t d) -> uint32_t {
      uint64_t acc = 0;
      for (uint32_t b = 0; b < r->n_batches; b++) {
        uint64_t rows = std::min<uint64_t>(r->batch, r->n_rows - (uint64_t)b * r->batch);
        acc += rows - co.null_counts[b];
        if (d < acc) return b;
      }
      return r->n_batches ? r->n_batches - 1 : 0;
    };
    int best_status = 0;
    uint32_t best_batch = 0xffffffffu;
    const PlainStream* cur_src = nullptr;
    const PlainStream* best_src = nullptr;
    bool best_eof = false;
    auto consider = [&](int code, uint32_t batch) {
      if (code && batch < best_batch) {
        best_batch = batch;
        best_status = code & ~(int)ORC_E_EOF;
        best_eof = (code & (int)ORC_E_EOF) || best_status == (int)ORC_E_IO;
        best_src = cur_src;
      }
    };
    int jl[4] = {cp.job_present, cp.job_data, cp.job_length, cp.job_secondary};
    unsigned long long fe = h_scalars[cp.err_idx];
    auto consider_fe = [&] {
      if (fe == RLE_NO_ERR) return;
      const bool dense_index = cp.c.orc_type == ORCGPU_T_FLOAT || cp.c.orc_type == ORCGPU_T_DOUBLE || cp.c.orc_type == ORCGPU_T_UNION;
      cur_src = &cp.data;
      const uint32_t b = dense_index ? batch_of_dense(fe >> 8) : (uint32_t)std::min<uint64_t>(r->n_batches ? r->n_batches - 1 : 0, (fe >> 8) / r->batch);
      consider((int)(fe & 0xff), b);
    };
    const PlainStream* ext_src = cp.is_dict ? &cp.dict : &cp.data;
    const PlainStream* job_src[4] = {&cp.present, &cp.data, &cp.length, &cp.secondary};
    auto consider_job = [&](int k) {
      if (jl[k] < 0) return;
      unsigned long long e = hjobs[P.jobs[jl[k]].final_index].err;
      if (e == RLE_NO_ERR) return;
      uint64_t idx = e >> 8;
      const uint64_t lead = P.jobs[jl[k]].skip_values;
      idx = idx > lead ? idx - lead : 0;
      int code = (int)(hjobs[P.jobs[jl[k]].final_index].err_pos & 0xff);
      if (k == 1 && cp.c.orc_type == ORCGPU_T_BOOLEAN) idx *= 8;
      cur_src = job_src[k];
      consider(code, resolve_job_batch(P, cp, co, r, k, idx, batch_of_dense));
    };
    auto consider_ext = [&] {
      cur_src = ext_src;
      resolve_ext(P, cp, co, r, h_scalars, h_chartot, consider);
    };
    if (cp.c.orc_type == ORCGPU_T_DECIMAL) {
      consider_ext();
      consider_fe();
      for (int k = 1; k < 4; k++) consider_job(k);
    } else if (cp.is_dict) {
      consider_job(2);
      consider_ext();
      consider_job(1);
      consider_fe();
    } else {
      for (int k = 1; k < 4; k++) consider_job(k);
      consider_fe();
      consider_ext();
    }
    if (best_status && best_eof && best_src && best_src->exists && best_src->err_idx) {
      const uint64_t ce = h_scalars[best_src->err_idx];
      if (ce == ORC_E_CODEC) best_status = ORCGPU_BUILD_DECODER;
      else if (ce == ORC_E_IO) best_status = ORCGPU_IO_ERROR;
    }
    co.status = best_status;
    co.err_batch = best_status ? best_batch : 0;
    if (cp.c.orc_type == ORCGPU_T_DECIMAL && cp.n_rows && r->n_batches) {
      const uint32_t pr = cp.c.precision & 0xffu;
      const int sc = (int8_t)cp.c.scale;
      if ((pr == 0 || pr > 38 || sc > 38 || (sc > 0 && (uint32_t)sc > pr)) && (!co.status || co.err_batch > 0)) {
        co.status = ORCGPU_ARROW;
        co.err_batch = 0;
      }
    }
  }
  if (host_prof) fprintf(stderr, "[orcgpu] lane %d host us: post %.1f  (call total %.1f)\n", ctx->lane_id, hclock() - ht_sync, hclock() - ht0);
  return ORCGPU_OK;
}

static int decode_staged_once(orcgpu_ctx* ctx, orcgpu_staged* const* stripes, uint32_t n, orcgpu_result** results);

extern "C" int orcgpu_decode_staged(orcgpu_ctx* ctx, orcgpu_staged* const* stripes, uint32_t n, orcgpu_result** results) {
  if (!ctx || !stripes || !results || !n) return ORCGPU_INVALID_ARGUMENT;
  int rc = decode_staged_once(ctx, stripes, n, results);
  if (rc == ORCGPU_RETRY_LARGER_SLOTS) rc = decode_staged_once(ctx, stripes, n, results);
  return rc == ORCGPU_RETRY_LARGER_SLOTS ? ORCGPU_UNEXPECTED : rc;
}

static int decode_staged_once(orcgpu_ctx* ctx, orcgpu_staged* const* stripes, uint32_t n, orcgpu_result** results) {
  const double call_t0 = std::chrono::duration<double, std::micro>(std::chrono::steady_clock::now().time_since_epoch()).count();
  HIP_TRY(ctx, hipSetDevice(ctx->device));
  for (uint32_t si = 0; si < n; si++) {
    orcgpu_staged* s = stripes[si];
    if (!s || s->ctx != ctx) return ORCGPU_INVALID_ARGUMENT;
    orcgpu_result* r = results[si];
    if (r && r->hold && orcgpu_hold::hold_exported(r->hold)) {
      set_err(ctx, "a result that exported device batches still view cannot be decoded into again");
      return ORCGPU_INVALID_ARGUMENT;
    }
    if (r && r->was_exported) {
      HIP_TRY(ctx, hipDeviceSynchronize());
      r->was_exported = false;
    }
    if (!r) {
      r = new orcgpu_result();
      results[si] = r;
    }
    r->ctx = ctx;
    r->n_rows = s->desc.n_rows;
    r->batch = s->desc.batch_size;
    r->n_batches = (uint32_t)((r->n_rows + r->batch - 1) / r->batch);
    r->words_per_batch = (r->batch + 63) / 64;
    r->cols.assign(s->cols.size(), ColumnOut{});
    for (size_t ci = 0; ci < s->cols.size(); ci++) {
      ColumnOut& co = r->cols[ci];
      co.column_id = s->cols[ci].column_id;
      co.orc_type = s->cols[ci].orc_type;
      const uint32_t par = s->cols[ci].parent;
      if (par && par <= ci) {
        co.parent = (int32_t)par - 1;
        const int pt = s->cols[par - 1].orc_type;
        co.elem = r->cols[par - 1].elem || pt == ORCGPU_T_LIST || pt == ORCGPU_T_MAP;
      }
    }
    for (auto* sub : r->subs) orcgpu_result_free(sub);
    r->subs.clear();
    r->status = 0;
    r->err_batch = r->err_col = 0;
    if (r->mirror) r->mirror->wait();
    r->mirror_valid = false;
    r->dev_ready_recorded = false;
    r->selected = false;
    r->sel.clear();
    r->filtered = false;
    r->filt_used = 0;
    for (int l = 0; l < kMaxLanes; l++) r->arena_used[l] = r->chars_used[l] = 0;
  }
  const int forced_lanes = [] {
    const char* e = getenv("ORCGPU_LANES");
    int v = e ? atoi(e) : 0;
    return v < 0 ? 0 : (v > kMaxLanes ? kMaxLanes : v);
  }();
  size_t max_cols = 0;
  for (uint32_t si = 0; si < n; si++) max_cols = std::max(max_cols, stripes[si]->cols.size());
  int want_lanes = forced_lanes ? forced_lanes : 1;
  if (!forced_lanes && max_cols >= 4) {
    uint64_t staged = 0;
    uint32_t mx_all = 0;
    for (uint32_t si = 0; si < n; si++)
      for (auto& st : stripes[si]->streams) {
        staged += st.len;
        for (auto& zp : st.zchunks)
          for (auto& it : zp.items) mx_all = std::max(mx_all, it.nseq);
      }
    if (staged >= (64ull << 20) && mx_all >= 16384) want_lanes = 2;
  }
  int n_lanes = (int)std::min<size_t>((size_t)want_lanes, max_cols);
  const bool auto_lanes = !forced_lanes && n_lanes > 1;
  std::vector<std::vector<std::vector<uint8_t>>> masks;
  int call_z = -1;
  auto root_id = [&](uint32_t si, uint32_t column_id) -> uint32_t {
    const auto& cols = stripes[si]->cols;
    size_t k = 0;
    for (; k < cols.size(); k++)
      if (cols[k].column_id == column_id) break;
    if (k == cols.size()) return column_id;
    while (cols[k].parent && cols[k].parent <= k) k = cols[k].parent - 1;
    return cols[k].column_id;
  };
  if (n_lanes > 1) {
    std::vector<std::pair<uint64_t, uint32_t>> w;
    uint64_t total = 0;
    for (uint32_t si = 0; si < n; si++)
      for (auto& c : stripes[si]->cols) {
        uint64_t b = 0;
        for (auto& st : stripes[si]->streams)
          if (st.column_id == c.column_id) b += st.len;
        const uint32_t rid = root_id(si, c.column_id);
        size_t k = 0;
        for (; k < w.size(); k++)
          if (w[k].second == rid) break;
        if (k == w.size()) w.push_back({0, rid});
        w[k].first += b;
        total += b;
      }
    std::sort(w.begin(), w.end(), [](auto& a, auto& b) { return a.first != b.first ? a.first > b.first : a.second < b.second; });
    std::vector<uint64_t> load(n_lanes, 0);
    std::vector<int> lane_of(w.size(), 0);
    std::vector<bool> closed(n_lanes, false);
    for (size_t k = 0; k < w.size(); k++) {
      int best = -1;
      for (int l = 0; l < n_lanes; l++)
        if (!closed[l] && (best < 0 || load[l] < load[best])) best = l;
      if (best < 0) best = 0;
      lane_of[k] = best;
      load[best] += w[k].first;
      if (k == 0 && w.size() > 1 && w[0].first * 4 >= total && n_lanes > 1) closed[best] = true;
    }
    {
      std::vector<uint32_t> mx(w.size(), 0);
      uint32_t mxmax = 0;
      for (uint32_t si = 0; si < n; si++)
        for (auto& st : stripes[si]->streams) {
          const uint32_t rid = root_id(si, st.column_id);
          size_t k = 0;
          for (; k < w.size(); k++)
            if (w[k].second == rid) break;
          if (k == w.size()) continue;
          for (auto& zp : st.zchunks)
            for (auto& it : zp.items) mx[k] = std::max(mx[k], it.nseq);
          mxmax = std::max(mxmax, mx[k]);
        }
      uint64_t seq_all = 0;
      for (uint32_t si = 0; si < n; si++)
        for (auto& st : stripes[si]->streams)
          for (auto& zp : st.zchunks)
            for (auto& it : zp.items) seq_all += it.nseq;
      const uint64_t lanes_min = kZstdLanesMinSequences;
      call_z = seq_all >= lanes_min ? 1 : 0;
      if (mxmax >= 4096 && n_lanes == 2 && seq_all >= lanes_min) {
        std::vector<uint64_t> lload(n_lanes, 0);
        const uint64_t handicap = 0;
        lload[0] = total * handicap / 1000;
        for (size_t k = 0; k < w.size(); k++)
          if (mx[k] * 5ull >= mxmax * 3ull) {
            lane_of[k] = 0;
            lload[0] += w[k].first;
          }
        for (size_t k = 0; k < w.size(); k++)
          if (mx[k] * 5ull < mxmax * 3ull) {
            const int best = lload[1] < lload[0] ? 1 : 0;
            lane_of[k] = best;
            lload[best] += w[k].first;
          }
      } else if (mxmax >= 4096) {
        std::vector<uint64_t> lload(n_lanes, 0);
        size_t heavy = 0;
        for (size_t k = 0; k < w.size(); k++) heavy += mx[k] * 2ull >= mxmax;
        if (heavy == w.size() && auto_lanes) n_lanes = 1;
        if (heavy < w.size())
          for (size_t k = 0; k < w.size(); k++) {
            if (mx[k] * 2ull >= mxmax) {
              lane_of[k] = 0;
            } else {
              int best = 1;
              for (int l = 2; l < n_lanes; l++)
                if (lload[l] < lload[best]) best = l;
              lane_of[k] = best;
              lload[best] += w[k].first;
            }
          }
      }
    }
    masks.assign(n_lanes, {});
    for (int l = 0; l < n_lanes; l++) {
      masks[l].resize(n);
      for (uint32_t si = 0; si < n; si++) {
        masks[l][si].assign(stripes[si]->cols.size(), 0);
        for (size_t ci = 0; ci < stripes[si]->cols.size(); ci++) {
          const uint32_t rid = root_id(si, stripes[si]->cols[ci].column_id);
          size_t k = 0;
          for (; k < w.size(); k++)
            if (w[k].second == rid) break;
          masks[l][si][ci] = lane_of[k] == l;
        }
      }
    }
    for (int l = n_lanes - 1; l >= 1; l--) {
      bool any = false;
      for (auto& m : masks[l])
        for (auto v : m) any |= v != 0;
      if (!any && l == n_lanes - 1) n_lanes--;
    }
  }
  int rc = ORCGPU_OK;
  ctx->call_t0 = call_t0;
  ctx->call_z_lanes = n_lanes > 1 ? call_z : -1;
  ctx->n_gate_peers = 0;
  ctx->tables_gate.store(0);
  const double t_pre = std::chrono::duration<double, std::micro>(std::chrono::steady_clock::now().time_since_epoch()).count();
  if (n_lanes <= 1) {
    rc = decode_lane(ctx, stripes, n, results, nullptr);
  } else {
    for (int l = 1; l < n_lanes; l++)
      if (!ctx->lanes[l]) {
        orcgpu_ctx* c = open_ctx(ctx->device, nullptr, l);
        if (!c) {
          set_err(ctx, "could not create lane %d", l);
          return ORCGPU_HIP_ERROR;
        }
        c->lane_id = l;
        ctx->lanes[l] = c;
      }
    for (int l = 1; l < n_lanes; l++) ctx->lanes[l]->call_t0 = call_t0;
    for (int l = 1; l < n_lanes; l++) ctx->lanes[l]->call_z_lanes = ctx->call_z_lanes;
    constexpr bool tables_first = true;
    for (int l = 0; l < n_lanes; l++) {
      orcgpu_ctx* c = ctx->lanes[l];
      c->tables_gate.store(0);
      c->n_gate_peers = 0;
// ... 85 lines not shown
          if (!par || par > k) continue;
          const bool child = par - 1 == ci, below = map_new[par - 1] != 0;
          if (!child && !below) continue;
          orcgpu_column c = s->cols[k];
          c.parent = child ? 0u : map_new[par - 1];
          v->cols.push_back(c);
          src.push_back(r->src_col.empty() ? (uint32_t)k : r->src_col[k]);
          map_new[k] = (uint32_t)v->cols.size();
        }
        for (auto& st : s->streams)
          for (auto& c : v->cols)
            if (c.column_id == st.column_id) {
              v->streams.push_back(st);
              v->stream_bytes += st.len;
              break;
            }
        orcgpu_result* sub = new orcgpu_result();
        sub->src_col = src;
        co.sub = (int32_t)r->subs.size();
        r->subs.push_back(sub);
        vptr.push_back(v.get());
        vres.push_back(sub);
        vst.push_back(std::move(v));
        owner.push_back(Owner{si, (uint32_t)ci});
      }
    }
    if (!vptr.empty()) {
      int rc2 = decode_staged_once(ctx, vptr.data(), (uint32_t)vptr.size(), vres.data());
      if (rc2 == ORCGPU_RETRY_LARGER_SLOTS) rc2 = decode_staged_once(ctx, vptr.data(), (uint32_t)vptr.size(), vres.data());
      for (auto& v : vst) v->dev = nullptr;
      if (rc2) return rc2 == ORCGPU_RETRY_LARGER_SLOTS ? ORCGPU_UNEXPECTED : rc2;
      for (size_t k = 0; k < vres.size(); k++) {
        orcgpu_result* r = results[owner[k].si];
        r->arrow_bytes += vres[k]->arrow_bytes;
        if (vres[k]->status && !r->status) {
          r->status = vres[k]->status;
          r->err_batch = 0;
          r->err_col = owner[k].col;
        }
        if (!r->status && r->cols[owner[k].col].orc_type == ORCGPU_T_MAP && !vres[k]->cols.empty()) {
          uint64_t key_nulls = 0;
          for (uint64_t c : vres[k]->cols[0].null_counts) key_nulls += c;
          if (key_nulls) {
            r->status = ORCGPU_ARROW;
            r->err_batch = 0;
            r->err_col = owner[k].col;
          }
        }
      }
    }
  }
  if (getenv("ORCGPU_DEBUG")) fprintf(stderr, "[orcgpu] call host us: behind the lanes %.1f\n", std::chrono::duration<double, std::micro>(std::chrono::steady_clock::now().time_since_epoch()).count() - t_lanes);
  return ORCGPU_OK;
}

extern "C" int orcgpu_stripe_decode(orcgpu_ctx* ctx, const orcgpu_stripe_desc* desc, orcgpu_result** out) {
  if (!out) return ORCGPU_INVALID_ARGUMENT;
  orcgpu_staged* s = nullptr;
  int rc = orcgpu_stage_stripe(ctx, desc, &s);
  if (rc) return rc;
  orcgpu_result* r = nullptr;
  rc = orcgpu_decode_staged(ctx, &s, 1, &r);
  orcgpu_staged_free(s);
  if (rc) {
    orcgpu_result_free(r);
    return rc;
  }
  *out = r;
  return ORCGPU_OK;
}

extern "C" int orcgpu_last_phase_ms(const orcgpu_ctx* ctx, float* ms, uint32_t n) {
  if (!ctx || !ms) return ORCGPU_INVALID_ARGUMENT;
  for (uint32_t k = 0; k < n && k < ORCGPU_N_PHASES; k++) ms[k] = ctx->last_phase_ms[k];
  return ORCGPU_OK;
}

extern "C" int orcgpu_last_lane_stats(const orcgpu_ctx* ctx, uint32_t lane, orcgpu_lane_stats* out) {
  if (!ctx || !out || lane >= ctx->last_n_lanes || lane >= (uint32_t)kMaxLanes || !ctx->lanes[lane]) return ORCGPU_INVALID_ARGUMENT;
  *out = ctx->lanes[lane]->last_stats;
  return ORCGPU_OK;
}

extern "C" int orcgpu_last_timing(const orcgpu_ctx* ctx, float* total_ms, float* expand_ms, uint32_t* expand_launches) {
  if (!ctx) return ORCGPU_INVALID_ARGUMENT;
  if (total_ms) *total_ms = ctx->last_total_ms;
  if (expand_ms) *expand_ms = ctx->last_expand_ms;
  if (expand_launches) *expand_launches = ctx->last_expand_launches;
  return ORCGPU_OK;
}
```

orc_rust_amd/csrc/orcgpu_decompress.inc:

```
namespace {

struct ZBlockPlan {
  uint32_t chunk;
  const ZItemH* item;
  const ZChunkParse* zp;
  uint64_t lit_off = ~0ull, seq_off = ~0ull;
  uint32_t zblock = 0;
};

template <class F>
std::vector<uint32_t> order_by_count_desc(uint32_t n, F count) {
  constexpr uint32_t kBuckets = 1u << 18;
  std::vector<uint32_t> key(n), at;
  uint32_t mx = 0, live = 0;
  for (uint32_t k = 0; k < n; k++) {
    const int64_t c = count(k);
    key[k] = c < 0 ? 0xffffffffu : (uint32_t)std::min<int64_t>(c, kBuckets - 1);
    if (c >= 0) mx = std::max(mx, key[k]), live++;
  }
  at.assign((size_t)mx + 2, 0);
  for (uint32_t k = 0; k < n; k++)
    if (key[k] != 0xffffffffu) at[mx - key[k] + 1]++;
  for (uint32_t b = 0; b <= mx; b++) at[b + 1] += at[b];
  std::vector<uint32_t> out(live);
  for (uint32_t k = 0; k < n; k++)
    if (key[k] != 0xffffffffu) out[at[mx - key[k]]++] = k;
  return out;
}

struct DecompPlan {
  uint64_t table_bytes = 0;
  uint64_t chunks_off = 0, streams_off = 0, zblocks_off = 0, zitems_off = 0;
  uint64_t dev_off = 0;
  uint32_t n_chunks = 0, n_streams = 0, n_zblocks = 0, n_zitems = 0;
  uint64_t zdump_off = 0;
  uint64_t zstatus_off = 0;
  uint64_t zprogress_off = 0;
  uint64_t order_off = 0;
  bool z_split_literals = false;
  bool z_lanes = false;
  uint64_t z_total_seq = 0;
  uint32_t n_zchains = 0;
  uint64_t ztab_off = 0, zhdr_off = 0;
  uint64_t chunk_start_off = 0;
  std::vector<ZBlockPlan> zitems;
  std::vector<uint32_t> chunk_first_item;
  std::vector<uint64_t> chunk_rec_off;
};

int plan_decompress(Plan& P, DecompPlan& DP) {
  if (P.decomp.empty()) return ORCGPU_OK;
  {
    size_t n_items = 0, n_chunks = 0;
    for (auto& ds : P.decomp) {
      n_chunks += ds.st->chunks.size();
      for (auto& zp : ds.st->zchunks) n_items += zp.items.size();
    }
    DP.zitems.reserve(n_items);
    DP.chunk_first_item.reserve(n_chunks);
    DP.chunk_rec_off.reserve(n_chunks);
  }
  for (auto& ds : P.decomp) {
    int k = ds.stripe->desc.compression;
    DP.n_streams++;
    for (auto& c : ds.st->chunks) {
      DP.chunk_first_item.push_back((uint32_t)DP.zitems.size());
      uint64_t rec = ~0ull;
      if (!c.original && k == ORCGPU_COMP_SNAPPY) rec = P.scratch.take(8ull * (c.len / 2 + 2), 16);
      else if (!c.original && k == ORCGPU_COMP_LZ4) rec = P.scratch.take(8ull * (2 * (c.len / 3 + 1) + 2), 16);
      else if (!c.original && k == ORCGPU_COMP_ZLIB) rec = P.scratch.take(((uint64_t)c.plain_cap + 16 + 15 & ~15ull) + 12ull * (c.plain_cap / 3 + 2) + 16, 16);
      DP.chunk_rec_off.push_back(rec);
      if (c.zparse >= 0) {
        const ZChunkParse& zp = ds.st->zchunks[c.zparse];
        for (auto& it : zp.items) {
          ZBlockPlan bp;
          bp.chunk = DP.n_chunks;
          bp.item = &it;
          bp.zp = &zp;
          if (it.kind == 2) {
            bp.zblock = DP.n_zblocks++;
            if (it.lit_type >= 2) bp.lit_off = P.scratch.take((uint64_t)it.lit_regen + 16, 16);
            if (it.nseq) bp.seq_off = P.scratch.take(12ull * ((it.nseq + 3u) & ~3u) + 16, 16);
          }
          DP.zitems.push_back(bp);
        }
      }
      DP.n_chunks++;
    }
  }
  DP.n_zitems = (uint32_t)DP.zitems.size();
  {
    std::vector<uint32_t> order = order_by_count_desc(DP.n_zitems, [&](uint32_t k) -> int64_t { return DP.zitems[k].item->kind == 2 ? (int64_t)DP.zitems[k].item->nseq : -1; });
    for (uint32_t r = 0; r < order.size(); r++) DP.zitems[order[r]].zblock = r;
    uint64_t total_seq = 0, longest = 0;
    for (uint32_t r = 0; r < order.size(); r++) {
      const uint64_t ns = DP.zitems[order[r]].item->nseq;
      total_seq += ns;
      longest = std::max(longest, ns);
      if (ns) DP.n_zchains++;
    }
    const char* force = getenv("ORCGPU_ZSTD_LANES");
    const uint64_t min_seq = kZstdLanesMinSequences;
    DP.z_lanes = DP.n_zchains && (force ? atoi(force) != 0 : (P.call_z_lanes >= 0 ? P.call_z_lanes != 0 : total_seq >= min_seq));
    DP.z_split_literals = DP.z_lanes;
    DP.z_total_seq = total_seq;
    (void)longest;
    if (DP.z_lanes) {
      DP.ztab_off = P.scratch.take((uint64_t)DP.n_zchains * ZL_CELLS * 2 + 16, 16);
      DP.zhdr_off = P.scratch.take((uint64_t)DP.n_zchains * sizeof(ZSeqHdr) + 16, 16);
    }
  }
  if (DP.n_zblocks) DP.zdump_off = P.scratch.take(1024 * 64 * 4);
  DP.zstatus_off = P.scratch.take(8ull * DP.n_zblocks + 16);
  DP.zprogress_off = P.scratch.take(4ull * DP.n_zblocks + 16);
  DP.chunk_start_off = P.scratch.take(4ull * DP.n_chunks + 16);
  Bump b;
  DP.chunks_off = b.take((uint64_t)DP.n_chunks * sizeof(ChunkDesc), 16);
  DP.streams_off = b.take((uint64_t)DP.n_streams * sizeof(StreamDesc), 16);
  DP.zblocks_off = b.take((uint64_t)DP.n_zblocks * sizeof(ZBlock), 16);
  DP.zitems_off = b.take((uint64_t)DP.n_zitems * sizeof(ZItem), 16);
  DP.order_off = b.take((uint64_t)DP.n_chunks * 4, 16);
  DP.table_bytes = align_up(b.off, 16);
  DP.dev_off = P.scratch.take(DP.table_bytes);
  return ORCGPU_OK;
}

static bool decomp_side_by_side(const orcgpu_ctx* ctx, const ChunkDesc* h_chunks, uint32_t n_chunks, uint32_t n_zblocks, bool z_lanes) {
  if (z_lanes) return false;
  constexpr bool use_inflate_parse = true;
  bool deflate = false;
  for (uint32_t i = 0; i < n_chunks; i++) deflate = deflate || h_chunks[i].kind == 1;
  return n_zblocks && ctx->aux_stream && !(deflate && use_inflate_parse);
}

static int launch_chunk_decoders(orcgpu_ctx* ctx, hipStream_t st, ChunkDesc* d_chunks, const ChunkDesc* h_chunks, uint32_t n_chunks, ZBlock* d_zblocks,
                                 uint32_t n_zblocks, const ZItem* d_zitems, uint32_t* d_zdump, uint32_t* d_zstatus, uint32_t* d_zprogress, const uint32_t* d_order, hipEvent_t stage1_done = nullptr,
                                 uint32_t n_zchains = 0, uint16_t* d_ztab = nullptr, ZSeqHdr* d_zhdr = nullptr, bool split_literals = false, hipEvent_t tables_ev = nullptr,
                                 hipEvent_t seq_done_ev = nullptr) {
  bool deflate = false, tokens = false, others = false, lzo = false;
  constexpr bool use_inflate_parse = true;
  for (uint32_t i = 0; i < n_chunks; i++) {
    const uint32_t k = h_chunks[i].kind;
    if (k == 1) deflate = true;
    else if (k == 3) lzo = true;
    else others = true;
    if (k == 2 || k == 4) tokens = true;
  }
  if (deflate && use_inflate_parse) others = true;
  int copy_too = 1;
  if (others) {
    const bool side = decomp_side_by_side(ctx, h_chunks, n_chunks, n_zblocks, d_ztab != nullptr);
    if (n_zblocks) HIP_TRY(ctx, hipMemsetAsync(d_zstatus, 0xff, 8ull * n_zblocks, st));
    HIP_TRY(ctx, hipMemsetAsync(d_zprogress, 0, 4ull * n_zblocks + 8, st));
    if (side) {
      HIP_TRY(ctx, hipEventRecord(ctx->aux_ev[0], st));
      HIP_TRY(ctx, hipStreamWaitEvent(ctx->aux_stream, ctx->aux_ev[0], 0));
    }
    const bool lit_aside = split_literals && d_ztab && ctx->aux_stream && !(getenv("ORCGPU_ZSTD_LIT_ASIDE") && atoi(getenv("ORCGPU_ZSTD_LIT_ASIDE")) == 0);
    if (n_zblocks && split_literals && !lit_aside)
      HIP_TRY(ctx, launch(zstd_literals_kernel, (uint64_t)n_zblocks, true, 64, st, (const ZBlock*)d_zblocks, n_zblocks, d_zstatus, d_zprogress));
    if (n_zblocks) HIP_TRY(ctx, launch(zstd_entropy_kernel, (split_literals ? 1ull : 2ull) * n_zblocks, true, 64, st, (const ZBlock*)d_zblocks, n_zblocks, d_zdump, d_zstatus, d_zprogress, d_ztab, d_zhdr));
    if (d_ztab && n_zchains) {
      if (tables_ev) HIP_TRY(ctx, hipEventRecord(tables_ev, st));
      if (tables_ev) ctx->tables_gate.store(1, std::memory_order_release);
      for (int k = 0; k < ctx->n_gate_peers; k++) {
        orcgpu_ctx* peer = ctx->gate_peers[k];
        int g = 0;
        for (int spins = 0; spins < 100000 && !(g = peer->tables_gate.load(std::memory_order_acquire)); spins++) std::this_thread::yield();
        if (g == 1) HIP_TRY(ctx, hipStreamWaitEvent(st, peer->ev[7], 0));
      }
      if (tables_ev) HIP_TRY(ctx, hipEventRecord(ctx->ev[9], st));
    }
    if (n_zblocks && lit_aside) HIP_TRY(ctx, hipEventRecord(ctx->aux_ev[0], st));
    if (d_ztab && n_zchains) {
      HIP_TRY(ctx, launch(zstd_seq_quads_kernel, (uint64_t)(n_zchains + 15) / 16, true, 64, st, (const ZBlock*)d_zblocks, n_zchains, (const uint16_t*)d_ztab, (const ZSeqHdr*)d_zhdr, d_zstatus));
      if (seq_done_ev) HIP_TRY(ctx, hipEventRecord(seq_done_ev, st));
    }
    if (n_zblocks && lit_aside) {
      HIP_TRY(ctx, hipStreamWaitEvent(ctx->aux_stream, ctx->aux_ev[0], 0));
      HIP_TRY(ctx, hipEventRecord(ctx->lit_ev[0], ctx->aux_stream));
      HIP_TRY(ctx, launch(zstd_literals_kernel, (uint64_t)n_zblocks, true, 64, ctx->aux_stream, (const ZBlock*)d_zblocks, n_zblocks, d_zstatus, d_zprogress));
      HIP_TRY(ctx, hipEventRecord(ctx->lit_ev[1], ctx->aux_stream));
      ctx->lit_ev_used = true;
      HIP_TRY(ctx, hipEventRecord(ctx->aux_ev[1], ctx->aux_stream));
      HIP_TRY(ctx, hipStreamWaitEvent(st, ctx->aux_ev[1], 0));
    }
    if (tokens) HIP_TRY(ctx, launch(lz_parse_kernel, (uint64_t)n_chunks, true, 64 * LZP_WAVES, st, d_chunks, n_chunks));
    if (deflate && use_inflate_parse) {
      const bool four = n_chunks <= 6u * (ctx->n_cus ? ctx->n_cus : 256u);
      ctx->dbg_inflate_threads = four ? 256u : 64u;
      if (four) {
        HIP_TRY(ctx, launch(inflate_parse4_kernel, (uint64_t)n_chunks, true, 256, st, d_chunks, n_chunks, 0u, 0xffffffffu));
      } else {
        HIP_TRY(ctx, launch(inflate_parse_kernel, (uint64_t)n_chunks, true, 64, st, d_chunks, n_chunks, 0u, 0xffffffffu));
      }
    }
    if (stage1_done) HIP_TRY(ctx, hipEventRecord(stage1_done, st));
    stage1_done = nullptr;
    if (tokens) {
      const bool four = n_chunks > 4u * (ctx->n_cus ? ctx->n_cus : 256u);
      if (four) HIP_TRY(ctx, launch(lz_exec_tokens4_kernel, (uint64_t)n_chunks, true, 256, st, d_chunks, n_chunks));
      else HIP_TRY(ctx, launch(lz_exec_tokens_kernel, (uint64_t)n_chunks, true, LZT_THREADS, st, d_chunks, n_chunks));
    }
    hipStream_t xs = side ? ctx->aux_stream : st;
    const char* pe = getenv("ORCGPU_EXEC_PATIENCE");
    const uint32_t patience = pe ? (uint32_t)atoll(pe) : (uint32_t)LZX_WATCHDOG;
    const uint64_t xgrid = std::min<uint64_t>(n_chunks, (side ? 512ull / LZX_THREADS : 1024ull / LZX_THREADS) * (ctx->n_cus ? ctx->n_cus : 256));
    const bool single_shot = d_ztab != nullptr || (!side && n_chunks >= 2048);
    const bool wave_groups = single_shot;
    if (deflate) ctx->dbg_exec_threads = wave_groups ? 64u : (uint32_t)LZX_THREADS;
    if (wave_groups)
      HIP_TRY(ctx, launch(lz_exec_wave_kernel, (uint64_t)n_chunks, true, 64, xs, d_chunks, n_chunks, d_zitems, (const ZBlock*)d_zblocks, (const uint32_t*)d_zstatus,
                          (const uint32_t*)d_zprogress, n_zblocks, copy_too, d_order));
    else
    HIP_TRY(ctx, launch(lz_exec_kernel, single_shot ? (uint64_t)n_chunks : xgrid, true, LZX_THREADS, xs, d_chunks, n_chunks, d_zitems, (const ZBlock*)d_zblocks, (const uint32_t*)d_zstatus,
                        (const uint32_t*)d_zprogress, n_zblocks, copy_too, d_order, single_shot ? (uint32_t*)nullptr : d_zprogress + n_zblocks, side ? 0 : 2, patience));
    if (side) {
      HIP_TRY(ctx, hipEventRecord(ctx->aux_ev[1], ctx->aux_stream));
      HIP_TRY(ctx, hipStreamWaitEvent(st, ctx->aux_ev[1], 0));
      const uint64_t xgrid2 = std::min<uint64_t>(n_chunks, (1024ull / LZX_THREADS) * (ctx->n_cus ? ctx->n_cus : 256));
      HIP_TRY(ctx, hipMemsetAsync(d_zprogress + n_zblocks, 0, 4, st));
      HIP_TRY(ctx, launch(lz_exec_kernel, xgrid2, true, LZX_THREADS, st, d_chunks, n_chunks, d_zitems, (const ZBlock*)d_zblocks, (const uint32_t*)d_zstatus,
                          (const uint32_t*)d_zprogress, n_zblocks, copy_too, d_order, d_zprogress + n_zblocks, 1, (uint32_t)LZX_WATCHDOG));
    }
    copy_too = 0;
  }
  if (stage1_done) HIP_TRY(ctx, hipEventRecord(stage1_done, st));
  if (lzo) {
    HIP_TRY(ctx, launch(decompress_lzo_kernel, (uint64_t)n_chunks, true, 64, st, d_chunks, n_chunks));
  }
  if (deflate) HIP_TRY(ctx, launch(decompress_deflate_kernel, (uint64_t)n_chunks, true, 64, st, d_chunks, n_chunks, copy_too, use_inflate_parse ? 1 : 0));
  return ORCGPU_OK;
}

int launch_decompress(orcgpu_ctx* ctx, Plan& P, DecompPlan& DP, uint8_t* S, uint64_t* d_scalars, uint8_t* host_blob, hipEvent_t stage1 = nullptr, hipEvent_t tables_ev = nullptr,
                      hipEvent_t done_ev = nullptr, hipEvent_t seq_done_ev = nullptr) {
  if (!(DP.z_lanes && DP.n_zchains && DP.n_chunks)) ctx->tables_gate.store(2, std::memory_order_release);
  if (tables_ev && !(DP.z_lanes && DP.n_zchains && DP.n_chunks)) HIP_TRY(ctx, hipEventRecord(tables_ev, ctx->stream));
  if (!DP.n_streams || !DP.n_chunks) {
    if (stage1) HIP_TRY(ctx, hipEventRecord(stage1, ctx->stream));
    if (!DP.n_streams) {
      if (done_ev) HIP_TRY(ctx, hipEventRecord(done_ev, ctx->stream));
      return ORCGPU_OK;
    }
    stage1 = nullptr;
  }
  hipStream_t st = ctx->stream;
  ChunkDesc* hc = reinterpret_cast<ChunkDesc*>(host_blob + DP.chunks_off);
  StreamDesc* hstr = reinterpret_cast<StreamDesc*>(host_blob + DP.streams_off);
  ZBlock* hzb = reinterpret_cast<ZBlock*>(host_blob + DP.zblocks_off);
  ZItem* hzi = reinterpret_cast<ZItem*>(host_blob + DP.zitems_off);
  auto fill_stream = [&](uint32_t si, uint32_t ci) {
    auto& ds = P.decomp[si];
    StreamDesc& sd = hstr[si];
    sd.first_chunk = ci;
    sd.n_chunks = (uint32_t)ds.st->chunks.size();
    sd.len_idx = ds.len_idx;
    sd.err_idx = ds.err_idx;
    sd.base = ds.result_index >= 0 ? P.results[ds.result_index]->arena[ctx->lane_id].p + ds.result_off : S + ds.scratch_off;
    sd.framing_error = ds.st->framing_error ? 1 : 0;
    sd.skip = ds.st->skip_bytes;
    uint64_t slot = 0;
    for (auto& c : ds.st->chunks) {
      ChunkDesc& cd = hc[ci];
      cd.src = ds.stripe->dev + ds.st->off + c.src_off;
      cd.dst = sd.base + slot;
      cd.scratch = DP.chunk_rec_off[ci] != ~0ull ? S + DP.chunk_rec_off[ci] : nullptr;
      cd.src_len = c.len;
      cd.dst_cap = c.plain_cap;
      cd.kind = c.original ? 0u : (uint32_t)ds.stripe->desc.compression;
      cd.stream = si;
      cd.out_len = 0;
      cd.status = 0;
      cd.first_item = DP.chunk_first_item[ci];
      cd.n_items = 0;
      cd.diag = 0;
      cd.pad = 0;
      if (c.zparse >= 0) {
        const ZChunkParse& zp = ds.st->zchunks[c.zparse];
        cd.n_items = (uint32_t)zp.items.size();
        if (zp.bad) cd.status = ORC_E_CODEC;
        for (uint32_t k = 0; k < cd.n_items; k++) {
          const ZBlockPlan& bp = DP.zitems[cd.first_item + k];
          const ZItemH& ih = *bp.item;
          ZItem& zi = hzi[cd.first_item + k];
          memset(&zi, 0, sizeof(zi));
          zi.kind = ih.kind;
          zi.flags = ih.flags;
          zi.fcs = ih.fcs;
          zi.ck_off = ih.ck_off;
          if (ih.kind == 0) {
            zi.size = ih.size;
            zi.src_off = ih.off;
          } else if (ih.kind == 1) {
            zi.size = ih.size;
            zi.src_off = ih.rle_byte;
          } else {
            zi.lit_kind = ih.lit_type == 0 ? 0u : (ih.lit_type == 1 ? 1u : 2u);
            zi.lit_off = ih.lit_type == 1 ? (uint32_t)ih.rle_byte : ih.off + ih.lit_hdr;
            zi.litn = ih.lit_regen;
            zi.nseq = ih.nseq;
            zi.zblock = bp.zblock;
            zi.seq_packed = DP.z_lanes ? 1u : 0u;
            ZBlock& zb = hzb[bp.zblock];
            memset(&zb, 0, sizeof(zb));
            zb.src = cd.src;
            zb.lit_out = bp.lit_off != ~0ull ? S + bp.lit_off : nullptr;
            zb.seq_out = bp.seq_off != ~0ull ? reinterpret_cast<uint32_t*>(S + bp.seq_off) : nullptr;
            zb.chunk = ci;
            zb.content_off = ih.off;
            zb.content_end = ih.off + ih.size;
            zb.lit_type = ih.lit_type;
            zb.lit_streams = ih.lit_streams;
            zb.lit_hdr = ih.lit_hdr;
            zb.lit_regen = ih.lit_regen;
            zb.lit_comp = ih.lit_comp;
            zb.nseq = ih.nseq;
            zb.seq_off = ih.seq_off;
            if (ih.lit_type == 3) {
              const ZItemH& def = zp.items[ih.huf_def];
              zb.huf_off = def.off + def.lit_hdr;
              zb.huf_end = zb.huf_off + def.lit_comp;
            }
            for (int w = 0; w < 3; w++) {
              const ZItemH& def = ih.nseq && ih.tab_def[w] >= 0 ? zp.items[ih.tab_def[w]] : ih;
              zb.tab_off[w] = def.seq_off;
              zb.tab_end[w] = def.off + def.size;
            }
          }
        }
      }
      slot += c.plain_cap;
      ci++;
    }
  };
  {
    const uint32_t ns = (uint32_t)P.decomp.size();
    std::vector<uint32_t> first(ns + 1, 0);
    for (uint32_t k = 0; k < ns; k++) first[k + 1] = first[k] + (uint32_t)P.decomp[k].st->chunks.size();
    const uint32_t nthreads = DP.n_zitems >= 8192 && ns >= 8 ? 4u : 1u;
    if (nthreads == 1) {
      for (uint32_t k = 0; k < ns; k++) fill_stream(k, first[k]);
    } else {
      std::vector<std::thread> th;
      uint32_t lo = 0;
      for (uint32_t t = 0; t < nthreads; t++) {
        uint32_t hi = lo;
        const uint32_t want = (uint32_t)((uint64_t)first[ns] * (t + 1) / nthreads);
        while (hi < ns && (first[hi + 1] <= want || t + 1 == nthreads)) hi++;
        if (t + 1 == nthreads) hi = ns;
        th.emplace_back([&, lo, hi] {
          for (uint32_t k = lo; k < hi; k++) fill_stream(k, first[k]);
        });
        lo = hi;
      }
      for (auto& x : th) x.join();
    }
  }
  if (decomp_side_by_side(ctx, hc, DP.n_chunks, DP.n_zblocks, DP.z_lanes))
    for (uint32_t c = 0; c < DP.n_chunks; c++)
      if (hc[c].kind == 5 || hc[c].kind == 0) hc[c].diag = LZX_DEFERRED;
  {
    uint32_t* ord = reinterpret_cast<uint32_t*>(host_blob + DP.order_off);
    const std::vector<uint32_t> by = order_by_count_desc(DP.n_chunks, [&](uint32_t c) -> int64_t {
      uint64_t ns = 0;
      const uint32_t f = DP.chunk_first_item[c], e = c + 1 < DP.n_chunks ? DP.chunk_first_item[c + 1] : DP.n_zitems;
      for (uint32_t k = f; k < e; k++) ns += DP.zitems[k].item->nseq;
      return (int64_t)ns;
    });
    for (uint32_t c = 0; c < DP.n_chunks; c++) ord[c] = by[c];
  }
  ChunkDesc* d_chunks = reinterpret_cast<ChunkDesc*>(S + DP.dev_off + DP.chunks_off);
  StreamDesc* d_streams = reinterpret_cast<StreamDesc*>(S + DP.dev_off + DP.streams_off);
  ZBlock* d_zblocks = reinterpret_cast<ZBlock*>(S + DP.dev_off + DP.zblocks_off);
  ZItem* d_zitems = reinterpret_cast<ZItem*>(S + DP.dev_off + DP.zitems_off);
  HIP_TRY(ctx, hipMemcpyAsync(S + DP.dev_off, host_blob, DP.table_bytes, hipMemcpyHostToDevice, st));
  if (DP.n_chunks) {
    int rc = launch_chunk_decoders(ctx, st, d_chunks, hc, DP.n_chunks, d_zblocks, DP.n_zblocks, d_zitems, reinterpret_cast<uint32_t*>(S + DP.zdump_off),
                                   reinterpret_cast<uint32_t*>(S + DP.zstatus_off), reinterpret_cast<uint32_t*>(S + DP.zprogress_off), reinterpret_cast<const uint32_t*>(S + DP.dev_off + DP.order_off), stage1,
                                   DP.n_zchains, DP.z_lanes ? reinterpret_cast<uint16_t*>(S + DP.ztab_off) : nullptr, DP.z_lanes ? reinterpret_cast<ZSeqHdr*>(S + DP.zhdr_off) : nullptr, DP.z_split_literals, tables_ev, seq_done_ev);
    if (rc) return rc;
  }
  if (done_ev) HIP_TRY(ctx, hipEventRecord(done_ev, st));
  HIP_TRY(ctx, launch(decompress_finalize_kernel, (uint64_t)DP.n_streams, true, 64, st, (const ChunkDesc*)d_chunks, (const StreamDesc*)d_streams, d_scalars,
                      reinterpret_cast<uint32_t*>(S + DP.chunk_start_off)));
  return ORCGPU_OK;
}

}
```

Baseline: 384.9.

## Precompute per-stream decompression tables at staging time and patch pointers at decode

Builds the ChunkDesc/ZItem/ZBlock tables, sequence counts, and chunk ordering once per staged stream when chunks are parsed. The per-call fill step then only rebases pointers and copies the prebuilt tables, replacing a multithreaded per-item rebuild and a separate sort by sequence count. Lane-selection heuristics read cached max and total sequence counts instead of rescanning every item. It also adds per-phase host timing counters and an API to read them, which costs a few clock reads per call and more host memory per staged stream.

```diff
diff --git a/include/orcgpu.h b/include/orcgpu.h
--- a/include/orcgpu.h
+++ b/include/orcgpu.h
@@ -337,6 +337,9 @@
 } orcgpu_lane_stats;
 int orcgpu_last_lane_stats(const orcgpu_ctx* ctx, uint32_t lane, orcgpu_lane_stats* out);
 
+#define ORCGPU_N_HOST_PARTS 11
+int orcgpu_last_lane_host_us(const orcgpu_ctx* ctx, uint32_t lane, float* us, uint32_t n);
+
 #ifdef __cplusplus
 }
 #endif
diff --git a/orc_rust_amd/capi.py b/orc_rust_amd/capi.py
--- a/orc_rust_amd/capi.py
+++ b/orc_rust_amd/capi.py
@@ -15,7 +15,7 @@
     "orcgpu_open", "orcgpu_close", "orcgpu_last_error", "orcgpu_version", "orcgpu_abi_version", "orcgpu_stage_stripe", "orcgpu_staged_free",
     "orcgpu_staged_bytes", "orcgpu_decode_staged", "orcgpu_stripe_decode", "orcgpu_result_free", "orcgpu_result_status",
     "orcgpu_result_rows", "orcgpu_result_batches", "orcgpu_result_arrow_bytes", "orcgpu_result_batch_view",
-    "orcgpu_result_copy_batch", "orcgpu_result_fetch", "orcgpu_result_fetch_async", "orcgpu_result_select", "orcgpu_selection_batches", "orcgpu_timezone_offsets", "orcgpu_result_export_batch", "orcgpu_last_timing", "orcgpu_last_phase_ms", "orcgpu_last_lane_stats", "orcgpu_encode_rle2_i64", "orcgpu_encode_rle2", "orcgpu_encode_byte_rle", "orcgpu_encode_boolean", "orcgpu_encode_column", "orcgpu_encode_fetch",
+    "orcgpu_result_copy_batch", "orcgpu_result_fetch", "orcgpu_result_fetch_async", "orcgpu_result_select", "orcgpu_selection_batches", "orcgpu_timezone_offsets", "orcgpu_result_export_batch", "orcgpu_last_timing", "orcgpu_last_phase_ms", "orcgpu_last_lane_stats", "orcgpu_last_lane_host_us", "orcgpu_encode_rle2_i64", "orcgpu_encode_rle2", "orcgpu_encode_byte_rle", "orcgpu_encode_boolean", "orcgpu_encode_column", "orcgpu_encode_fetch",
     "orcgpu_reader_open_file", "orcgpu_reader_open_bytes", "orcgpu_reader_close", "orcgpu_reader_set_batch_size",
     "orcgpu_reader_set_projection", "orcgpu_reader_set_projection_roots", "orcgpu_reader_set_schema", "orcgpu_reader_set_byte_range", "orcgpu_reader_set_shard", "orcgpu_shard_columns", "orcgpu_reader_column_weight", "orcgpu_reader_set_timestamp_precision", "orcgpu_reader_set_row_selection", "orcgpu_reader_set_prefetch",
     "orcgpu_reader_set_row_group_pruning", "orcgpu_reader_row_groups", "orcgpu_index_entry", "orcgpu_reader_set_predicate",
@@ -201,6 +201,7 @@
     L.orcgpu_last_timing.argtypes = [C.c_void_p, C.POINTER(C.c_float), C.POINTER(C.c_float), C.POINTER(C.c_uint32)]
     L.orcgpu_last_phase_ms.argtypes = [C.c_void_p, C.POINTER(C.c_float), C.c_uint32]
     L.orcgpu_last_lane_stats.argtypes = [C.c_void_p, C.c_uint32, C.POINTER(LaneStats)]
+    L.orcgpu_last_lane_host_us.argtypes = [C.c_void_p, C.c_uint32, C.POINTER(C.c_float), C.c_uint32]
     L.orcgpu_encode_rle2_i64.argtypes = [C.c_void_p, C.c_void_p, C.c_uint64, C.c_int, C.c_void_p, C.c_uint64, C.POINTER(C.c_uint64)]
     L.orcgpu_encode_rle2.argtypes = [C.c_void_p, C.c_void_p, C.c_uint64, C.c_int, C.c_int, C.c_uint32, C.c_void_p, C.c_uint64, C.POINTER(C.c_uint64)]
     L.orcgpu_encode_byte_rle.argtypes = [C.c_void_p, C.c_void_p, C.c_uint64, C.c_uint32, C.c_void_p, C.c_uint64, C.POINTER(C.c_uint64)]
@@ -434,6 +435,15 @@
                 break
         return out
 
+    HOST_PARTS = ("lanes", "columns", "chunks", "layout", "fill", "upload", "gate", "decomp", "enqueue", "wait", "summary")
+
+    def lane_host_us(self):
+        out = []
+        a = (C.c_float * len(self.HOST_PARTS))()
+        while len(out) < 4 and self.L.orcgpu_last_lane_host_us(self.h, len(out), a, len(self.HOST_PARTS)) == OK:
+            out.append(dict(zip(self.HOST_PARTS, [float(x) for x in a])))
+        return out
+
 
 class Staged:
     def __init__(self, ctx, h):
diff --git a/orc_rust_amd/csrc/device/decomp_tables.h b/orc_rust_amd/csrc/device/decomp_tables.h
--- /dev/null
+++ b/orc_rust_amd/csrc/device/decomp_tables.h
@@ -0,0 +1,61 @@
+#pragma once
+#include <cstdint>
+
+struct ChunkDesc {
+  const uint8_t* src;
+  uint8_t* dst;
+  uint8_t* scratch;
+  uint32_t src_len;
+  uint32_t dst_cap;
+  uint32_t kind;
+  uint32_t stream;
+  uint32_t out_len;
+  uint32_t status;
+  uint32_t first_item, n_items;
+  uint32_t diag;
+  uint32_t pad;
+};
+
+struct StreamDesc {
+  uint32_t first_chunk, n_chunks;
+  uint32_t len_idx;
+  uint32_t err_idx;
+  uint8_t* base;
+  uint32_t framing_error;
+  uint32_t skip;
+};
+
+struct ZBlock {
+  const uint8_t* src;
+  uint8_t* lit_out;
+  uint32_t* seq_out;
+  uint32_t chunk;
+  uint32_t content_off, content_end;
+  uint32_t lit_type, lit_streams, lit_hdr, lit_regen, lit_comp;
+  uint32_t nseq, seq_off;
+  uint32_t huf_off, huf_end;
+  uint32_t tab_off[3];
+  uint32_t tab_end[3];
+  uint32_t pad[2];
+};
+
+struct ZSeqHdr {
+  uint32_t bit_off;
+  uint32_t logs;
+  uint32_t status;
+  uint32_t pad;
+};
+
+struct ZItem {
+  uint32_t kind;
+  uint32_t flags;
+  uint32_t size;
+  uint32_t src_off;
+  uint32_t lit_kind;
+  uint32_t lit_off, litn, nseq;
+  uint32_t zblock;
+  uint32_t seq_packed;
+  uint64_t fcs;
+  uint32_t ck_off;
+  uint32_t pad;
+};
diff --git a/orc_rust_amd/csrc/device/decompress_kernels.hip b/orc_rust_amd/csrc/device/decompress_kernels.hip
--- a/orc_rust_amd/csrc/device/decompress_kernels.hip
+++ b/orc_rust_amd/csrc/device/decompress_kernels.hip
@@ -1,29 +1,7 @@
 #pragma once
 #include "rle_parse.h"
 
-struct ChunkDesc {
-  const uint8_t* src;
-  uint8_t* dst;
-  uint8_t* scratch;
-  uint32_t src_len;
-  uint32_t dst_cap;
-  uint32_t kind;
-  uint32_t stream;
-  uint32_t out_len;
-  uint32_t status;
-  uint32_t first_item, n_items;
-  uint32_t diag;
-  uint32_t pad;
-};
-
-struct StreamDesc {
-  uint32_t first_chunk, n_chunks;
-  uint32_t len_idx;
-  uint32_t err_idx;
-  uint8_t* base;
-  uint32_t framing_error;
-  uint32_t skip;
-};
+#include "decomp_tables.h"
 
 __device__ __forceinline__ void wave_fence() { __builtin_amdgcn_fence(__ATOMIC_SEQ_CST, "workgroup"); }
 __device__ __forceinline__ void lds_order() {
diff --git a/orc_rust_amd/csrc/device/lz_exec.h b/orc_rust_amd/csrc/device/lz_exec.h
--- a/orc_rust_amd/csrc/device/lz_exec.h
+++ b/orc_rust_amd/csrc/device/lz_exec.h
@@ -11,19 +11,7 @@
 #define LZX_SEQ_PACKED 0xffffffffu
 #define LZX_DEFERRED 0x57a7u
 
-struct ZItem {
-  uint32_t kind;
-  uint32_t flags;
-  uint32_t size;
-  uint32_t src_off;
-  uint32_t lit_kind;
-  uint32_t lit_off, litn, nseq;
-  uint32_t zblock;
-  uint32_t seq_packed;
-  uint64_t fcs;
-  uint32_t ck_off;
-  uint32_t pad;
-};
+#include "decomp_tables.h"
 
 template <int T>
 struct ExecLds {
diff --git a/orc_rust_amd/csrc/device/zstd_entropy.h b/orc_rust_amd/csrc/device/zstd_entropy.h
--- a/orc_rust_amd/csrc/device/zstd_entropy.h
+++ b/orc_rust_amd/csrc/device/zstd_entropy.h
@@ -1,25 +1,7 @@
 #pragma once
 
-struct ZBlock {
-  const uint8_t* src;
-  uint8_t* lit_out;
-  uint32_t* seq_out;
-  uint32_t chunk;
-  uint32_t content_off, content_end;
-  uint32_t lit_type, lit_streams, lit_hdr, lit_regen, lit_comp;
-  uint32_t nseq, seq_off;
-  uint32_t huf_off, huf_end;
-  uint32_t tab_off[3];
-  uint32_t tab_end[3];
-  uint32_t pad[2];
-};
-
-struct ZSeqHdr {
-  uint32_t bit_off;
-  uint32_t logs;
-  uint32_t status;
-  uint32_t pad;
-};
+#include "decomp_tables.h"
+
 __device__ __forceinline__ uint2 zseq_pack(uint32_t ofv, uint32_t ml, uint32_t ll) {
   const uint32_t o = ofv < 0x1fffffffu ? ofv : 0x1fffffffu;
   return make_uint2(o | ml << 29, ml >> 3 | ll << 15);
diff --git a/orc_rust_amd/csrc/orcgpu.hip b/orc_rust_amd/csrc/orcgpu.hip
--- a/orc_rust_amd/csrc/orcgpu.hip
+++ b/orc_rust_amd/csrc/orcgpu.hip
@@ -81,18 +81,11 @@
   }
 };
 
-struct ChunkInfo {
-  uint64_t src_off;
-  uint32_t len;
-  uint32_t original;
-  uint32_t plain_cap;
-  int32_t zparse = -1;
-};
-
 
 }
 
 #include "orcgpu_zstd_host.inc"
+#include "orcgpu_decomp_plan.inc"
 #include "orcgpu_tz.inc"
 
 namespace {
@@ -103,6 +96,7 @@
   uint64_t len;
   std::vector<ChunkInfo> chunks;
   std::vector<ZChunkParse> zchunks;
+  StreamTables tables;
   uint32_t skip_bytes = 0, skip_values = 0, skip_bits = 0;
   std::vector<std::pair<uint32_t, uint32_t>> hints;
   bool framing_error = false;
@@ -224,6 +218,8 @@
   orcgpu_lane_stats last_stats{};
   uint32_t last_n_lanes = 1;
   double call_t0 = 0;
+  float last_host_us[ORCGPU_N_HOST_PARTS] = {};
+  double hp_fill = 0, hp_upload = 0, hp_gate = 0;
   orcgpu_ctx* gate_peers[kMaxLanes] = {nullptr, nullptr, nullptr, nullptr};
   int n_gate_peers = 0;
 int call_z_lanes = -1;
@@ -522,6 +518,7 @@
     p += 3 + (uint64_t)len;
   }
   st.framed_len = p;
+  build_stream_tables(st.chunks, st.zchunks, compression, st.off, ORC_E_CODEC, st.tables);
 }
 
 uint32_t type_width(int t) {
diff --git a/orc_rust_amd/csrc/orcgpu_decode.inc b/orc_rust_amd/csrc/orcgpu_decode.inc
--- a/orc_rust_amd/csrc/orcgpu_decode.inc
+++ b/orc_rust_amd/csrc/orcgpu_decode.inc
@@ -508,6 +508,8 @@
   ctx->kev_used[0] = ctx->kev_used[1] = false;
   ctx->lit_ev_used = false;
   HIP_TRY(ctx, hipMemcpyAsync(dsum, hs, SL.bytes, hipMemcpyHostToDevice, st));
+  const double ht_launch = hclock();
+  ctx->hp_fill = ctx->hp_upload = ctx->hp_gate = 0;
   rc = launch_decompress(ctx, P, DP, S, d_scalars, hs + SL.bytes, ctx->ev[6], ctx->ev[7], ctx->ev[4], ctx->ev[8]);
   const double ht_first = hclock();
   if (rc) return rc;
@@ -850,11 +852,12 @@
   if (getenv("ORCGPU_DEBUG") && DP.n_zitems) {
     fprintf(stderr, "[orcgpu] zstd plan: %u blocks, %u with sequences (%llu in all): %s\n", DP.n_zblocks, DP.n_zchains, (unsigned long long)DP.z_total_seq,
             DP.z_lanes ? "one lane per block" : "one wavefront per block");
+    const ChunkDesc* tc = reinterpret_cast<const ChunkDesc*>(hs + SL.bytes + DP.chunks_off);
+    const ZItem* ti = reinterpret_cast<const ZItem*>(hs + SL.bytes + DP.zitems_off);
     std::vector<std::pair<uint64_t, uint32_t>> top;
     for (uint32_t c = 0; c < DP.n_chunks; c++) {
       uint64_t ns = 0;
-      const uint32_t f = DP.chunk_first_item[c], e = c + 1 < DP.n_chunks ? DP.chunk_first_item[c + 1] : DP.n_zitems;
-      for (uint32_t k = f; k < e; k++) ns += DP.zitems[k].item->nseq;
+      for (uint32_t k = tc[c].first_item; k < tc[c].first_item + tc[c].n_items; k++) ns += ti[k].nseq;
       top.push_back({ns, c});
     }
     std::sort(top.rbegin(), top.rend());
@@ -864,9 +867,9 @@
       fprintf(stderr, "[orcgpu] zstd chunks: %zu; with >= 40k / 20k / 10k / 5k sequences: %zu / %zu / %zu / %zu\n", top.size(), h40, h20, h10, h5);
     }
     for (size_t k = 0; k < top.size() && k < 6; k++) {
-      const uint32_t c = top[k].second, f = DP.chunk_first_item[c], e = c + 1 < DP.n_chunks ? DP.chunk_first_item[c + 1] : DP.n_zitems;
+      const uint32_t c = top[k].second, f = tc[c].first_item, e = f + tc[c].n_items;
       uint32_t mxs = 0, lit = 0;
-      for (uint32_t q = f; q < e; q++) mxs = std::max(mxs, DP.zitems[q].item->nseq), lit += DP.zitems[q].item->lit_regen;
+      for (uint32_t q = f; q < e; q++) mxs = std::max(mxs, ti[q].nseq), lit += ti[q].litn;
       fprintf(stderr, "[orcgpu] zstd chunk %u: %u blocks, %llu sequences (largest block %u), %u literal bytes\n", c, e - f, (unsigned long long)top[k].first, mxs, lit);
     }
   }
@@ -924,15 +927,17 @@
       for (auto& ds : P.decomp) {
         const int kind = ds.stripe->desc.compression;
         const uint64_t limit = std::max<uint64_t>(ds.stripe->desc.block_size, 1u << 22);
+        bool grown_here = false;
         for (auto& c : const_cast<StagedStream*>(ds.st)->chunks) {
           const bool grows = kind == ORCGPU_COMP_ZLIB || kind == ORCGPU_COMP_LZO ||
                              (kind == ORCGPU_COMP_ZSTD && c.zparse >= 0 && !ds.st->zchunks[c.zparse].size_known && !ds.st->zchunks[c.zparse].bad);
           if (!c.original && grows && hc[ci].status && c.plain_cap < limit) {
             c.plain_cap = (uint32_t)limit;
-            grown = true;
+            grown = grown_here = true;
           }
           ci++;
         }
+        if (grown_here) build_stream_tables(ds.st->chunks, ds.st->zchunks, kind, ds.st->off, ORC_E_CODEC, const_cast<StagedStream*>(ds.st)->tables);
       }
       if (grown) return ORCGPU_RETRY_LARGER_SLOTS;
     }
@@ -1025,6 +1030,11 @@
     }
   }
   if (host_prof) fprintf(stderr, "[orcgpu] lane %d host us: post %.1f  (call total %.1f)\n", ctx->lane_id, hclock() - ht_sync, hclock() - ht0);
+  {
+    const double parts[ORCGPU_N_HOST_PARTS] = {ctx->call_t0 > 0 ? ht0 - ctx->call_t0 : 0.0, ht_cols - ht0, ht_dp - ht_cols, ht_plan - ht_dp, ctx->hp_fill, ctx->hp_upload + (ht_launch - ht_plan),
+                                               ctx->hp_gate, (ht_first - ht_launch) - ctx->hp_fill - ctx->hp_upload - ctx->hp_gate, ht_enq - ht_first, ht_sync - ht_enq, hclock() - ht_sync};
+    for (int k = 0; k < ORCGPU_N_HOST_PARTS; k++) ctx->last_host_us[k] = (float)parts[k];
+  }
   return ORCGPU_OK;
 }
 
@@ -1100,8 +1110,7 @@
     for (uint32_t si = 0; si < n; si++)
       for (auto& st : stripes[si]->streams) {
         staged += st.len;
-        for (auto& zp : st.zchunks)
-          for (auto& it : zp.items) mx_all = std::max(mx_all, it.nseq);
+        mx_all = std::max(mx_all, st.tables.max_nseq);
       }
     if (staged >= (64ull << 20) && mx_all >= 16384) want_lanes = 2;
   }
@@ -1157,15 +1166,12 @@
           for (; k < w.size(); k++)
             if (w[k].second == rid) break;
           if (k == w.size()) continue;
-          for (auto& zp : st.zchunks)
-            for (auto& it : zp.items) mx[k] = std::max(mx[k], it.nseq);
+          mx[k] = std::max(mx[k], st.tables.max_nseq);
           mxmax = std::max(mxmax, mx[k]);
         }
       uint64_t seq_all = 0;
       for (uint32_t si = 0; si < n; si++)
-        for (auto& st : stripes[si]->streams)
-          for (auto& zp : st.zchunks)
-            for (auto& it : zp.items) seq_all += it.nseq;
+        for (auto& st : stripes[si]->streams) seq_all += st.tables.total_seq;
       const uint64_t lanes_min = kZstdLanesMinSequences;
       call_z = seq_all >= lanes_min ? 1 : 0;
       if (mxmax >= 4096 && n_lanes == 2 && seq_all >= lanes_min) {
@@ -1417,6 +1423,12 @@
   return ORCGPU_OK;
 }
 
+extern "C" int orcgpu_last_lane_host_us(const orcgpu_ctx* ctx, uint32_t lane, float* us, uint32_t n) {
+  if (!ctx || !us || lane >= ctx->last_n_lanes || lane >= (uint32_t)kMaxLanes || !ctx->lanes[lane]) return ORCGPU_INVALID_ARGUMENT;
+  for (uint32_t k = 0; k < n && k < ORCGPU_N_HOST_PARTS; k++) us[k] = ctx->lanes[lane]->last_host_us[k];
+  return ORCGPU_OK;
+}
+
 extern "C" int orcgpu_last_timing(const orcgpu_ctx* ctx, float* total_ms, float* expand_ms, uint32_t* expand_launches) {
   if (!ctx) return ORCGPU_INVALID_ARGUMENT;
   if (total_ms) *total_ms = ctx->last_total_ms;
diff --git a/orc_rust_amd/csrc/orcgpu_decomp_plan.inc b/orc_rust_amd/csrc/orcgpu_decomp_plan.inc
--- /dev/null
+++ b/orc_rust_amd/csrc/orcgpu_decomp_plan.inc
@@ -0,0 +1,279 @@
+#include <algorithm>
+#include <cstdint>
+#include <cstring>
+#include <utility>
+#include <vector>
+
+#include "device/decomp_tables.h"
+
+namespace {
+
+struct ChunkInfo {
+  uint64_t src_off;
+  uint32_t len;
+  uint32_t original;
+  uint32_t plain_cap;
+  int32_t zparse = -1;
+};
+
+constexpr uint32_t kCountBuckets = 1u << 18;
+inline uint32_t count_key(uint64_t c) { return (uint32_t)std::min<uint64_t>(c, kCountBuckets - 1); }
+
+inline uint64_t chunk_record_bytes(int compression, const ChunkInfo& c) {
+  if (c.original) return 0;
+  if (compression == ORCGPU_COMP_SNAPPY) return 8ull * (c.len / 2 + 2);
+  if (compression == ORCGPU_COMP_LZ4) return 8ull * (2 * (c.len / 3 + 1) + 2);
+  if (compression == ORCGPU_COMP_ZLIB) return (((uint64_t)c.plain_cap + 16 + 15) & ~15ull) + 12ull * (c.plain_cap / 3 + 2) + 16;
+  return 0;
+}
+
+constexpr uint32_t kSeqBytesArrays = 12, kSeqBytesPacked = 8;
+inline uint32_t seq_round(uint32_t nseq) { return (nseq + 3u) & ~3u; }
+
+struct StreamTables {
+  std::vector<ChunkDesc> chunks;
+  std::vector<ZItem> items;
+  std::vector<ZBlock> zblocks;
+  std::vector<uint32_t> zb_item;
+  std::vector<uint64_t> zb_seq_before;
+  std::vector<std::pair<uint32_t, uint32_t>> zb_hist;
+  std::vector<uint32_t> chunk_order;
+  std::vector<std::pair<uint32_t, uint32_t>> chunk_hist;
+  uint32_t n_chains = 0;
+  uint32_t max_nseq = 0;
+  uint64_t total_seq = 0;
+  uint64_t seq_rounded = 0;
+  uint64_t scratch8 = 0;
+  uint64_t plain_cap = 0;
+  uint64_t scratch_bytes(uint32_t seq_bytes) const { return scratch8 + (uint64_t)(seq_bytes - kSeqBytesPacked) * seq_rounded; }
+};
+
+void build_stream_tables(const std::vector<ChunkInfo>& chunks, const std::vector<ZChunkParse>& zchunks, int compression, uint64_t arena_off, uint32_t codec_error,
+                         StreamTables& T) {
+  T = StreamTables{};
+  T.chunks.reserve(chunks.size());
+  {
+    size_t n_items = 0;
+    for (auto& zp : zchunks) n_items += zp.items.size();
+    T.items.reserve(n_items);
+  }
+  auto rel = [](uint64_t v) { return reinterpret_cast<uint8_t*>((uintptr_t)v); };
+  std::vector<ZBlock> zb_pos;
+  std::vector<uint32_t> zb_pos_item;
+  std::vector<uint64_t> zb_pos_before;
+  std::vector<uint32_t> chunk_keys;
+  uint64_t slot = 0, sc = 0;
+  auto take = [&](uint64_t n) {
+    sc = (sc + 15) & ~15ull;
+    const uint64_t r = sc;
+    sc += n;
+    return r;
+  };
+  for (auto& c : chunks) {
+    const uint32_t ci = (uint32_t)T.chunks.size();
+    ChunkDesc cd;
+    memset(&cd, 0, sizeof(cd));
+    cd.src = rel(arena_off + c.src_off);
+    cd.dst = rel(slot);
+    const uint64_t rec = chunk_record_bytes(compression, c);
+    if (rec) cd.scratch = rel(take(rec) + 1);
+    cd.src_len = c.len;
+    cd.dst_cap = c.plain_cap;
+    cd.kind = c.original ? 0u : (uint32_t)compression;
+    cd.first_item = (uint32_t)T.items.size();
+    uint64_t chunk_seq = 0;
+    if (c.zparse >= 0) {
+      const ZChunkParse& zp = zchunks[c.zparse];
+      cd.n_items = (uint32_t)zp.items.size();
+      if (zp.bad) cd.status = codec_error;
+      for (const ZItemH& ih : zp.items) {
+        ZItem zi;
+        memset(&zi, 0, sizeof(zi));
+        zi.kind = ih.kind;
+        zi.flags = ih.flags;
+        zi.fcs = ih.fcs;
+        zi.ck_off = ih.ck_off;
+        if (ih.kind == 0) {
+          zi.size = ih.size;
+          zi.src_off = ih.off;
+        } else if (ih.kind == 1) {
+          zi.size = ih.size;
+          zi.src_off = ih.rle_byte;
+        } else {
+          zi.lit_kind = ih.lit_type == 0 ? 0u : (ih.lit_type == 1 ? 1u : 2u);
+          zi.lit_off = ih.lit_type == 1 ? (uint32_t)ih.rle_byte : ih.off + ih.lit_hdr;
+          zi.litn = ih.lit_regen;
+          zi.nseq = ih.nseq;
+          ZBlock zb;
+          memset(&zb, 0, sizeof(zb));
+          zb.src = cd.src;
+          zb_pos_before.push_back(T.seq_rounded);
+          if (ih.lit_type >= 2) zb.lit_out = rel(take((uint64_t)ih.lit_regen + 16) + 1);
+          if (ih.nseq) {
+            zb.seq_out = reinterpret_cast<uint32_t*>(rel(take((uint64_t)kSeqBytesPacked * seq_round(ih.nseq) + 16) + 1));
+            T.seq_rounded += seq_round(ih.nseq);
+            T.n_chains++;
+          }
+          zb.chunk = ci;
+          zb.content_off = ih.off;
+          zb.content_end = ih.off + ih.size;
+          zb.lit_type = ih.lit_type;
+          zb.lit_streams = ih.lit_streams;
+          zb.lit_hdr = ih.lit_hdr;
+          zb.lit_regen = ih.lit_regen;
+          zb.lit_comp = ih.lit_comp;
+          zb.nseq = ih.nseq;
+          zb.seq_off = ih.seq_off;
+          if (ih.lit_type == 3) {
+            const ZItemH& def = zp.items[ih.huf_def];
+            zb.huf_off = def.off + def.lit_hdr;
+            zb.huf_end = zb.huf_off + def.lit_comp;
+          }
+          for (int w = 0; w < 3; w++) {
+            const ZItemH& def = ih.nseq && ih.tab_def[w] >= 0 ? zp.items[ih.tab_def[w]] : ih;
+            zb.tab_off[w] = def.seq_off;
+            zb.tab_end[w] = def.off + def.size;
+          }
+          zb_pos.push_back(zb);
+          zb_pos_item.push_back((uint32_t)T.items.size());
+          chunk_seq += ih.nseq;
+          T.total_seq += ih.nseq;
+          T.max_nseq = std::max(T.max_nseq, ih.nseq);
+        }
+        T.items.push_back(zi);
+      }
+    }
+    chunk_keys.push_back(count_key(chunk_seq));
+    T.chunks.push_back(cd);
+    slot += c.plain_cap;
+  }
+  T.plain_cap = slot;
+  T.scratch8 = sc;
+  auto order_desc = [](uint32_t n, auto key, std::vector<uint32_t>& order, std::vector<std::pair<uint32_t, uint32_t>>& hist) {
+    order.resize(n);
+    for (uint32_t k = 0; k < n; k++) order[k] = k;
+    std::stable_sort(order.begin(), order.end(), [&](uint32_t a, uint32_t b) { return key(a) > key(b); });
+    hist.clear();
+    for (uint32_t k = 0; k < n; k++) {
+      if (hist.empty() || hist.back().first != key(order[k])) hist.push_back({key(order[k]), 0u});
+      hist.back().second++;
+    }
+  };
+  std::vector<uint32_t> zorder;
+  order_desc((uint32_t)zb_pos.size(), [&](uint32_t k) { return count_key(zb_pos[k].nseq); }, zorder, T.zb_hist);
+  T.zblocks.reserve(zorder.size());
+  T.zb_item.reserve(zorder.size());
+  T.zb_seq_before.reserve(zorder.size());
+  for (uint32_t k : zorder) {
+    T.zblocks.push_back(zb_pos[k]);
+    T.zb_item.push_back(zb_pos_item[k]);
+    T.zb_seq_before.push_back(zb_pos_before[k]);
+  }
+  order_desc((uint32_t)T.chunks.size(), [&](uint32_t k) { return chunk_keys[k]; }, T.chunk_order, T.chunk_hist);
+}
+
+struct TableCounts {
+  uint32_t n_streams = 0, n_chunks = 0, n_zblocks = 0, n_zitems = 0, n_zchains = 0;
+  uint64_t total_seq = 0;
+  std::vector<uint32_t> chunk0, item0;
+  std::vector<uint32_t> zb_at;
+  std::vector<uint32_t> chunk_at;
+};
+
+inline void ranks_of(const std::vector<std::pair<uint32_t, uint32_t>>* const* hists, size_t n, std::vector<uint32_t>& at) {
+  uint32_t mx = 0;
+  for (size_t k = 0; k < n; k++)
+    if (!hists[k]->empty()) mx = std::max(mx, hists[k]->front().first);
+  at.assign((size_t)mx + 1, 0);
+  for (size_t k = 0; k < n; k++)
+    for (auto& h : *hists[k]) at[h.first] += h.second;
+  uint32_t r = 0;
+  for (size_t key = at.size(); key-- > 0;) {
+    const uint32_t c = at[key];
+    at[key] = r;
+    r += c;
+  }
+}
+void tables_count(const StreamTables* const* t, size_t n, TableCounts& C) {
+  C = TableCounts{};
+  C.n_streams = (uint32_t)n;
+  C.chunk0.resize(n);
+  C.item0.resize(n);
+  std::vector<const std::vector<std::pair<uint32_t, uint32_t>>*> zh(n), ch(n);
+  for (size_t k = 0; k < n; k++) {
+    C.chunk0[k] = C.n_chunks;
+    C.item0[k] = C.n_zitems;
+    C.n_chunks += (uint32_t)t[k]->chunks.size();
+    C.n_zitems += (uint32_t)t[k]->items.size();
+    C.n_zblocks += (uint32_t)t[k]->zblocks.size();
+    C.n_zchains += t[k]->n_chains;
+    C.total_seq += t[k]->total_seq;
+    zh[k] = &t[k]->zb_hist;
+    ch[k] = &t[k]->chunk_hist;
+  }
+  ranks_of(zh.data(), n, C.zb_at);
+  ranks_of(ch.data(), n, C.chunk_at);
+}
+
+struct StreamUse {
+  const StreamTables* t;
+  const uint8_t* arena;
+  uint8_t* plain;
+  uint8_t* scratch;
+  uint32_t len_idx, err_idx, framing_error, skip;
+};
+
+void tables_fill(const StreamUse* use, const TableCounts& C, bool packed, ChunkDesc* hc, StreamDesc* hstr, ZBlock* hzb, ZItem* hzi, uint32_t* ord) {
+  std::vector<uint32_t> zb_at = C.zb_at, chunk_at = C.chunk_at;
+  const uint64_t extra = packed ? 0u : kSeqBytesArrays - kSeqBytesPacked;
+  auto at = [](const void* base, const void* rel, uint64_t more = 0) { return (uintptr_t)base + (uintptr_t)rel + (uintptr_t)more; };
+  for (uint32_t si = 0; si < C.n_streams; si++) {
+    const StreamUse& u = use[si];
+    const StreamTables& T = *u.t;
+    const uint32_t c0 = C.chunk0[si], i0 = C.item0[si];
+    StreamDesc& sd = hstr[si];
+    sd.first_chunk = c0;
+    sd.n_chunks = (uint32_t)T.chunks.size();
+    sd.len_idx = u.len_idx;
+    sd.err_idx = u.err_idx;
+    sd.base = u.plain;
+    sd.framing_error = u.framing_error;
+    sd.skip = u.skip;
+    const size_t nc = T.chunks.size();
+    if (nc) memcpy(hc + c0, T.chunks.data(), nc * sizeof(ChunkDesc));
+    for (size_t k = 0; k < nc; k++) {
+      ChunkDesc& cd = hc[c0 + k];
+      cd.src = reinterpret_cast<const uint8_t*>(at(u.arena, cd.src));
+      cd.dst = reinterpret_cast<uint8_t*>(at(u.plain, cd.dst));
+      if (cd.scratch) cd.scratch = reinterpret_cast<uint8_t*>(at(u.scratch, cd.scratch) - 1);
+      cd.stream = si;
+      cd.first_item += i0;
+    }
+    if (!T.items.empty()) memcpy(hzi + i0, T.items.data(), T.items.size() * sizeof(ZItem));
+    size_t j = 0;
+    for (auto& h : T.zb_hist) {
+      const uint32_t r0 = zb_at[h.first];
+      zb_at[h.first] += h.second;
+      memcpy(hzb + r0, T.zblocks.data() + j, (size_t)h.second * sizeof(ZBlock));
+      for (uint32_t q = 0; q < h.second; q++, j++) {
+        ZBlock& zb = hzb[r0 + q];
+        const uint64_t more = extra * T.zb_seq_before[j];
+        zb.src = reinterpret_cast<const uint8_t*>(at(u.arena, zb.src));
+        if (zb.lit_out) zb.lit_out = reinterpret_cast<uint8_t*>(at(u.scratch, zb.lit_out, more) - 1);
+        if (zb.seq_out) zb.seq_out = reinterpret_cast<uint32_t*>(at(u.scratch, zb.seq_out, more) - 1);
+        zb.chunk += c0;
+        ZItem& zi = hzi[i0 + T.zb_item[j]];
+        zi.zblock = r0 + q;
+        zi.seq_packed = packed ? 1u : 0u;
+      }
+    }
+    j = 0;
+    for (auto& h : T.chunk_hist) {
+      const uint32_t r0 = chunk_at[h.first];
+      chunk_at[h.first] += h.second;
+      for (uint32_t q = 0; q < h.second; q++, j++) ord[r0 + q] = c0 + T.chunk_order[j];
+    }
+  }
+}
+
+}
diff --git a/orc_rust_amd/csrc/orcgpu_decompress.inc b/orc_rust_amd/csrc/orcgpu_decompress.inc
--- a/orc_rust_amd/csrc/orcgpu_decompress.inc
+++ b/orc_rust_amd/csrc/orcgpu_decompress.inc
@@ -1,32 +1,6 @@
 namespace {
 
-struct ZBlockPlan {
-  uint32_t chunk;
-  const ZItemH* item;
-  const ZChunkParse* zp;
-  uint64_t lit_off = ~0ull, seq_off = ~0ull;
-  uint32_t zblock = 0;
-};
-
-template <class F>
-std::vector<uint32_t> order_by_count_desc(uint32_t n, F count) {
-  constexpr uint32_t kBuckets = 1u << 18;
-  std::vector<uint32_t> key(n), at;
-  uint32_t mx = 0, live = 0;
-  for (uint32_t k = 0; k < n; k++) {
-    const int64_t c = count(k);
-    key[k] = c < 0 ? 0xffffffffu : (uint32_t)std::min<int64_t>(c, kBuckets - 1);
-    if (c >= 0) mx = std::max(mx, key[k]), live++;
-  }
-  at.assign((size_t)mx + 2, 0);
-  for (uint32_t k = 0; k < n; k++)
-    if (key[k] != 0xffffffffu) at[mx - key[k] + 1]++;
-  for (uint32_t b = 0; b <= mx; b++) at[b + 1] += at[b];
-  std::vector<uint32_t> out(live);
-  for (uint32_t k = 0; k < n; k++)
-    if (key[k] != 0xffffffffu) out[at[mx - key[k]]++] = k;
-  return out;
-}
+inline double host_us_now() { return std::chrono::duration<double, std::micro>(std::chrono::steady_clock::now().time_since_epoch()).count(); }
 
 struct DecompPlan {
   uint64_t table_bytes = 0;
@@ -43,72 +17,40 @@
   uint32_t n_zchains = 0;
   uint64_t ztab_off = 0, zhdr_off = 0;
   uint64_t chunk_start_off = 0;
-  std::vector<ZBlockPlan> zitems;
-  std::vector<uint32_t> chunk_first_item;
-  std::vector<uint64_t> chunk_rec_off;
+  TableCounts counts;
+  std::vector<uint64_t> stream_scratch;
 };
 
 int plan_decompress(Plan& P, DecompPlan& DP) {
   if (P.decomp.empty()) return ORCGPU_OK;
+  const size_t ns = P.decomp.size();
   {
-    size_t n_items = 0, n_chunks = 0;
-    for (auto& ds : P.decomp) {
-      n_chunks += ds.st->chunks.size();
-      for (auto& zp : ds.st->zchunks) n_items += zp.items.size();
-    }
-    DP.zitems.reserve(n_items);
-    DP.chunk_first_item.reserve(n_chunks);
-    DP.chunk_rec_off.reserve(n_chunks);
-  }
-  for (auto& ds : P.decomp) {
-    int k = ds.stripe->desc.compression;
-    DP.n_streams++;
-    for (auto& c : ds.st->chunks) {
-      DP.chunk_first_item.push_back((uint32_t)DP.zitems.size());
-      uint64_t rec = ~0ull;
-      if (!c.original && k == ORCGPU_COMP_SNAPPY) rec = P.scratch.take(8ull * (c.len / 2 + 2), 16);
-      else if (!c.original && k == ORCGPU_COMP_LZ4) rec = P.scratch.take(8ull * (2 * (c.len / 3 + 1) + 2), 16);
-      else if (!c.original && k == ORCGPU_COMP_ZLIB) rec = P.scratch.take(((uint64_t)c.plain_cap + 16 + 15 & ~15ull) + 12ull * (c.plain_cap / 3 + 2) + 16, 16);
-      DP.chunk_rec_off.push_back(rec);
-      if (c.zparse >= 0) {
-        const ZChunkParse& zp = ds.st->zchunks[c.zparse];
-        for (auto& it : zp.items) {
-          ZBlockPlan bp;
-          bp.chunk = DP.n_chunks;
-          bp.item = &it;
-          bp.zp = &zp;
-          if (it.kind == 2) {
-            bp.zblock = DP.n_zblocks++;
-            if (it.lit_type >= 2) bp.lit_off = P.scratch.take((uint64_t)it.lit_regen + 16, 16);
-            if (it.nseq) bp.seq_off = P.scratch.take(12ull * ((it.nseq + 3u) & ~3u) + 16, 16);
-          }
-          DP.zitems.push_back(bp);
-        }
-      }
-      DP.n_chunks++;
-    }
-  }
-  DP.n_zitems = (uint32_t)DP.zitems.size();
+    std::vector<const StreamTables*> t(ns);
+    for (size_t k = 0; k < ns; k++) t[k] = &P.decomp[k].st->tables;
+    tables_count(t.data(), ns, DP.counts);
+  }
+  const TableCounts& C = DP.counts;
+  DP.n_streams = C.n_streams;
+  DP.n_chunks = C.n_chunks;
+  DP.n_zblocks = C.n_zblocks;
+  DP.n_zitems = C.n_zitems;
+  DP.n_zchains = C.n_zchains;
+  DP.z_total_seq = C.total_seq;
   {
-    std::vector<uint32_t> order = order_by_count_desc(DP.n_zitems, [&](uint32_t k) -> int64_t { return DP.zitems[k].item->kind == 2 ? (int64_t)DP.zitems[k].item->nseq : -1; });
-    for (uint32_t r = 0; r < order.size(); r++) DP.zitems[order[r]].zblock = r;
-    uint64_t total_seq = 0, longest = 0;
-    for (uint32_t r = 0; r < order.size(); r++) {
-      const uint64_t ns = DP.zitems[order[r]].item->nseq;
-      total_seq += ns;
-      longest = std::max(longest, ns);
-      if (ns) DP.n_zchains++;
-    }
     const char* force = getenv("ORCGPU_ZSTD_LANES");
     const uint64_t min_seq = kZstdLanesMinSequences;
-    DP.z_lanes = DP.n_zchains && (force ? atoi(force) != 0 : (P.call_z_lanes >= 0 ? P.call_z_lanes != 0 : total_seq >= min_seq));
+    DP.z_lanes = DP.n_zchains && (force ? atoi(force) != 0 : (P.call_z_lanes >= 0 ? P.call_z_lanes != 0 : C.total_seq >= min_seq));
     DP.z_split_literals = DP.z_lanes;
-    DP.z_total_seq = total_seq;
-    (void)longest;
-    if (DP.z_lanes) {
-      DP.ztab_off = P.scratch.take((uint64_t)DP.n_zchains * ZL_CELLS * 2 + 16, 16);
-      DP.zhdr_off = P.scratch.take((uint64_t)DP.n_zchains * sizeof(ZSeqHdr) + 16, 16);
-    }
+  }
+  DP.stream_scratch.assign(ns, ~0ull);
+  const uint32_t seq_bytes = DP.z_lanes ? kSeqBytesPacked : kSeqBytesArrays;
+  for (size_t k = 0; k < ns; k++) {
+    const uint64_t need = P.decomp[k].st->tables.scratch_bytes(seq_bytes);
+    if (need) DP.stream_scratch[k] = P.scratch.take(need, 16);
+  }
+  if (DP.z_lanes) {
+    DP.ztab_off = P.scratch.take((uint64_t)DP.n_zchains * ZL_CELLS * 2 + 16, 16);
+    DP.zhdr_off = P.scratch.take((uint64_t)DP.n_zchains * sizeof(ZSeqHdr) + 16, 16);
   }
   if (DP.n_zblocks) DP.zdump_off = P.scratch.take(1024 * 64 * 4);
   DP.zstatus_off = P.scratch.take(8ull * DP.n_zblocks + 16);
@@ -163,12 +105,14 @@
     if (d_ztab && n_zchains) {
       if (tables_ev) HIP_TRY(ctx, hipEventRecord(tables_ev, st));
       if (tables_ev) ctx->tables_gate.store(1, std::memory_order_release);
+      const double t_gate = host_us_now();
       for (int k = 0; k < ctx->n_gate_peers; k++) {
         orcgpu_ctx* peer = ctx->gate_peers[k];
         int g = 0;
         for (int spins = 0; spins < 100000 && !(g = peer->tables_gate.load(std::memory_order_acquire)); spins++) std::this_thread::yield();
         if (g == 1) HIP_TRY(ctx, hipStreamWaitEvent(st, peer->ev[7], 0));
       }
+      ctx->hp_gate += host_us_now() - t_gate;
       if (tables_ev) HIP_TRY(ctx, hipEventRecord(ctx->ev[9], st));
     }
     if (n_zblocks && lit_aside) HIP_TRY(ctx, hipEventRecord(ctx->aux_ev[0], st));
@@ -246,135 +190,38 @@
     stage1 = nullptr;
   }
   hipStream_t st = ctx->stream;
+  const double t_fill = host_us_now();
   ChunkDesc* hc = reinterpret_cast<ChunkDesc*>(host_blob + DP.chunks_off);
   StreamDesc* hstr = reinterpret_cast<StreamDesc*>(host_blob + DP.streams_off);
   ZBlock* hzb = reinterpret_cast<ZBlock*>(host_blob + DP.zblocks_off);
   ZItem* hzi = reinterpret_cast<ZItem*>(host_blob + DP.zitems_off);
-  auto fill_stream = [&](uint32_t si, uint32_t ci) {
-    auto& ds = P.decomp[si];
-    StreamDesc& sd = hstr[si];
-    sd.first_chunk = ci;
-    sd.n_chunks = (uint32_t)ds.st->chunks.size();
-    sd.len_idx = ds.len_idx;
-    sd.err_idx = ds.err_idx;
-    sd.base = ds.result_index >= 0 ? P.results[ds.result_index]->arena[ctx->lane_id].p + ds.result_off : S + ds.scratch_off;
-    sd.framing_error = ds.st->framing_error ? 1 : 0;
-    sd.skip = ds.st->skip_bytes;
-    uint64_t slot = 0;
-    for (auto& c : ds.st->chunks) {
-      ChunkDesc& cd = hc[ci];
-      cd.src = ds.stripe->dev + ds.st->off + c.src_off;
-      cd.dst = sd.base + slot;
-      cd.scratch = DP.chunk_rec_off[ci] != ~0ull ? S + DP.chunk_rec_off[ci] : nullptr;
-      cd.src_len = c.len;
-      cd.dst_cap = c.plain_cap;
-      cd.kind = c.original ? 0u : (uint32_t)ds.stripe->desc.compression;
-      cd.stream = si;
-      cd.out_len = 0;
-      cd.status = 0;
-      cd.first_item = DP.chunk_first_item[ci];
-      cd.n_items = 0;
-      cd.diag = 0;
-      cd.pad = 0;
-      if (c.zparse >= 0) {
-        const ZChunkParse& zp = ds.st->zchunks[c.zparse];
-        cd.n_items = (uint32_t)zp.items.size();
-        if (zp.bad) cd.status = ORC_E_CODEC;
-        for (uint32_t k = 0; k < cd.n_items; k++) {
-          const ZBlockPlan& bp = DP.zitems[cd.first_item + k];
-          const ZItemH& ih = *bp.item;
-          ZItem& zi = hzi[cd.first_item + k];
-          memset(&zi, 0, sizeof(zi));
-          zi.kind = ih.kind;
-          zi.flags = ih.flags;
-          zi.fcs = ih.fcs;
-          zi.ck_off = ih.ck_off;
-          if (ih.kind == 0) {
-            zi.size = ih.size;
-            zi.src_off = ih.off;
-          } else if (ih.kind == 1) {
-            zi.size = ih.size;
-            zi.src_off = ih.rle_byte;
-          } else {
-            zi.lit_kind = ih.lit_type == 0 ? 0u : (ih.lit_type == 1 ? 1u : 2u);
-            zi.lit_off = ih.lit_type == 1 ? (uint32_t)ih.rle_byte : ih.off + ih.lit_hdr;
-            zi.litn = ih.lit_regen;
-            zi.nseq = ih.nseq;
-            zi.zblock = bp.zblock;
-            zi.seq_packed = DP.z_lanes ? 1u : 0u;
-            ZBlock& zb = hzb[bp.zblock];
-            memset(&zb, 0, sizeof(zb));
-            zb.src = cd.src;
-            zb.lit_out = bp.lit_off != ~0ull ? S + bp.lit_off : nullptr;
-            zb.seq_out = bp.seq_off != ~0ull ? reinterpret_cast<uint32_t*>(S + bp.seq_off) : nullptr;
-            zb.chunk = ci;
-            zb.content_off = ih.off;
-            zb.content_end = ih.off + ih.size;
-            zb.lit_type = ih.lit_type;
-            zb.lit_streams = ih.lit_streams;
-            zb.lit_hdr = ih.lit_hdr;
-            zb.lit_regen = ih.lit_regen;
-            zb.lit_comp = ih.lit_comp;
-            zb.nseq = ih.nseq;
-            zb.seq_off = ih.seq_off;
-            if (ih.lit_type == 3) {
-              const ZItemH& def = zp.items[ih.huf_def];
-              zb.huf_off = def.off + def.lit_hdr;
-              zb.huf_end = zb.huf_off + def.lit_comp;
-            }
-            for (int w = 0; w < 3; w++) {
-              const ZItemH& def = ih.nseq && ih.tab_def[w] >= 0 ? zp.items[ih.tab_def[w]] : ih;
-              zb.tab_off[w] = def.seq_off;
-              zb.tab_end[w] = def.off + def.size;
-            }
-          }
-        }
-      }
-      slot += c.plain_cap;
-      ci++;
-    }
-  };
   {
-    const uint32_t ns = (uint32_t)P.decomp.size();
-    std::vector<uint32_t> first(ns + 1, 0);
-    for (uint32_t k = 0; k < ns; k++) first[k + 1] = first[k] + (uint32_t)P.decomp[k].st->chunks.size();
-    const uint32_t nthreads = DP.n_zitems >= 8192 && ns >= 8 ? 4u : 1u;
-    if (nthreads == 1) {
-      for (uint32_t k = 0; k < ns; k++) fill_stream(k, first[k]);
-    } else {
-      std::vector<std::thread> th;
-      uint32_t lo = 0;
-      for (uint32_t t = 0; t < nthreads; t++) {
-        uint32_t hi = lo;
-        const uint32_t want = (uint32_t)((uint64_t)first[ns] * (t + 1) / nthreads);
-        while (hi < ns && (first[hi + 1] <= want || t + 1 == nthreads)) hi++;
-        if (t + 1 == nthreads) hi = ns;
-        th.emplace_back([&, lo, hi] {
-          for (uint32_t k = lo; k < hi; k++) fill_stream(k, first[k]);
-        });
-        lo = hi;
-      }
-      for (auto& x : th) x.join();
-    }
+    std::vector<StreamUse> use(P.decomp.size());
+    for (size_t si = 0; si < use.size(); si++) {
+      const DecompStream& ds = P.decomp[si];
+      StreamUse& u = use[si];
+      u.t = &ds.st->tables;
+      u.arena = ds.stripe->dev;
+      u.plain = ds.result_index >= 0 ? P.results[ds.result_index]->arena[ctx->lane_id].p + ds.result_off : S + ds.scratch_off;
+      u.scratch = DP.stream_scratch[si] != ~0ull ? S + DP.stream_scratch[si] : nullptr;
+      u.len_idx = ds.len_idx;
+      u.err_idx = ds.err_idx;
+      u.framing_error = ds.st->framing_error ? 1 : 0;
+      u.skip = ds.st->skip_bytes;
+    }
+    tables_fill(use.data(), DP.counts, DP.z_lanes, hc, hstr, hzb, hzi, reinterpret_cast<uint32_t*>(host_blob + DP.order_off));
   }
   if (decomp_side_by_side(ctx, hc, DP.n_chunks, DP.n_zblocks, DP.z_lanes))
     for (uint32_t c = 0; c < DP.n_chunks; c++)
       if (hc[c].kind == 5 || hc[c].kind == 0) hc[c].diag = LZX_DEFERRED;
-  {
-    uint32_t* ord = reinterpret_cast<uint32_t*>(host_blob + DP.order_off);
-    const std::vector<uint32_t> by = order_by_count_desc(DP.n_chunks, [&](uint32_t c) -> int64_t {
-      uint64_t ns = 0;
-      const uint32_t f = DP.chunk_first_item[c], e = c + 1 < DP.n_chunks ? DP.chunk_first_item[c + 1] : DP.n_zitems;
-      for (uint32_t k = f; k < e; k++) ns += DP.zitems[k].item->nseq;
-      return (int64_t)ns;
-    });
-    for (uint32_t c = 0; c < DP.n_chunks; c++) ord[c] = by[c];
-  }
   ChunkDesc* d_chunks = reinterpret_cast<ChunkDesc*>(S + DP.dev_off + DP.chunks_off);
   StreamDesc* d_streams = reinterpret_cast<StreamDesc*>(S + DP.dev_off + DP.streams_off);
   ZBlock* d_zblocks = reinterpret_cast<ZBlock*>(S + DP.dev_off + DP.zblocks_off);
   ZItem* d_zitems = reinterpret_cast<ZItem*>(S + DP.dev_off + DP.zitems_off);
+  const double t_up = host_us_now();
+  ctx->hp_fill += t_up - t_fill;
   HIP_TRY(ctx, hipMemcpyAsync(S + DP.dev_off, host_blob, DP.table_bytes, hipMemcpyHostToDevice, st));
+  ctx->hp_upload += host_us_now() - t_up;
   if (DP.n_chunks) {
     int rc = launch_chunk_decoders(ctx, st, d_chunks, hc, DP.n_chunks, d_zblocks, DP.n_zblocks, d_zitems, reinterpret_cast<uint32_t*>(S + DP.zdump_off),
                                    reinterpret_cast<uint32_t*>(S + DP.zstatus_off), reinterpret_cast<uint32_t*>(S + DP.zprogress_off), reinterpret_cast<const uint32_t*>(S + DP.dev_off + DP.order_off), stage1,
diff --git a/profiles/host_breakdown.py b/profiles/host_breakdown.py
--- /dev/null
+++ b/profiles/host_breakdown.py
@@ -0,0 +1,35 @@
+import json
+import os
+import sys
+
+ROOT = os.path.dirname(os.path.dirname(os.path.abspath(__file__)))
+sys.path.insert(0, ROOT)
+
+import bench
+from orc_rust_amd import capi
+
+acc, steps = [], [0]
+_lane_stats = capi.Context.lane_stats
+
+
+def lane_stats(self):
+    for k, parts in enumerate(self.lane_host_us()):
+        if k == len(acc):
+            acc.append(dict.fromkeys(capi.Context.HOST_PARTS, 0.0))
+        for name, us in parts.items():
+            acc[k][name] += us
+    steps[0] += 1
+    return _lane_stats(self)
+
+
+capi.Context.lane_stats = lane_stats
+bench.main()
+n = max(1, steps[0])
+lanes = []
+for k, a in enumerate(acc):
+    d = {name: round(us / n, 1) for name, us in a.items()}
+    d["lane"] = k
+    d["before_first_launch_us"] = round(sum(a[p] for p in ("lanes", "columns", "chunks", "layout")) / n, 1)
+    d["tables_us"] = round(sum(a[p] for p in ("chunks", "fill", "upload")) / n, 1)
+    lanes.append(d)
+print(json.dumps({"host_us_per_step": lanes, "steps": steps[0]}))
```

Result: faster. 392.0, median of 6 (+1.8%).
